# martinambrus/PitchExtractor

Measured on AMD Instinct MI355X. Metric: mel-frames/sec training throughput (JDCNet, 24 kHz, batch=256), higher is better.
Workload: dtype f32

## Files before the change

### include/pitchextractor_hip.h

```cpp
#ifndef PITCHEXTRACTOR_HIP_H
#define PITCHEXTRACTOR_HIP_H

#include <stddef.h>
#include <stdint.h>

#ifdef __cplusplus
extern "C" {
#endif

#define PE_OK 0
#define PE_E_ARG (-1)
#define PE_E_UNSUPPORTED (-2)
#define PE_E_WORKSPACE (-3)

enum pe_products {
  PE_PROD_NATIVE = 0,
  PE_PROD_X3 = 1,
  PE_PROD_H2 = 2,
  PE_PROD_BF16 = 3,
  PE_PROD_F16 = 4
};

int pe_abi_version(void);
int pe_device_count(void);
int pe_stream_create_low_priority(void** stream_out);

typedef struct pe_mel_plan pe_mel_plan;
int pe_mel_plan_create(pe_mel_plan** plan, int sample_rate, int n_fft, int win_length,
                       int hop_length, int n_mels, float f_min, float f_max);
int pe_mel_plan_destroy(pe_mel_plan* plan);
int pe_mel_num_frames(const pe_mel_plan* plan, int n_samples);
int pe_mel_forward(const pe_mel_plan* plan, const float* wave, int batch, int n_samples,
                   long wave_stride, float* out, long out_sb, long out_sm, long out_st,
                   int out_frames, int log_mode, float log_eps, float mean, float std,
                   float pad_value, void* stream);
int pe_mel_forward_ragged(const pe_mel_plan* plan, const float* wave, int batch, int max_samples,
                          long wave_stride, const int* n_samples, const int* frame_start, float* out,
                          long out_sb, long out_sm, long out_st, int out_frames, int log_mode,
                          float log_eps, float mean, float std, float pad_value, void* stream);
int pe_mel_chunk_fields(void);
int pe_mel_forward_chunks(const pe_mel_plan* plan, const float* wave, long wave_elems, const long* chunks,
                          const long* host_chunks, int n_chunks, int chunk_size, float* out, long out_sb,
                          long out_sm, long out_st, int log_mode, float log_eps, float mean, float std,
                          float pad_value, void* stream);
size_t pe_mel_backward_workspace_bytes(const pe_mel_plan* plan, int batch, int max_samples, int out_frames);
int pe_mel_backward(const pe_mel_plan* plan, const float* wave, int batch, int n_samples, long wave_stride,
                    const float* grad_out, long g_sb, long g_sm, long g_st, int out_frames, int log_mode,
                    float log_eps, float mean, float std, float* grad_wave, long grad_wave_stride,
                    void* workspace, size_t workspace_bytes, void* stream);
int pe_mel_backward_ragged(const pe_mel_plan* plan, const float* wave, int batch, int max_samples,
                           long wave_stride, const int* n_samples, const int* frame_start,
                           const float* grad_out, long g_sb, long g_sm, long g_st, int out_frames,
                           int log_mode, float log_eps, float mean, float std, float* grad_wave,
                           long grad_wave_stride, void* workspace, size_t workspace_bytes, void* stream);

int pe_stitch_run_fields(void);
int pe_stitch_chunks(const float* x, long ld_x, const float* det, const long* runs, const long* host_runs,
                     int n_runs, int n_chunks, int chunk_size, int C, float* out, long ld_out, float* det_out,
                     long n_dst, void* stream);


int pe_gemm_nt(int products, int act16, const void* A, long lda, const float* B, long ldb, void* C, long ldc, int M,
               int N, int K, const float* bias0, const float* bias1, int accumulate, const unsigned* amax_a,
               const unsigned* amax_b, void* stream);
int pe_absmax(const float* x, long rows, int cols, long ld, unsigned* out, void* stream);
int pe_absmax_segments(const float* base, const long* seg_off, const long* seg_len, int nseg, unsigned* out,
                       void* stream);
size_t pe_gemm_tn_workspace_bytes(int M, int N, int K);
int pe_gemm_tn(int products, int act16, const void* A, long lda, const void* B, long ldb, float* C, long ldc, int M,
               int N, int K, int accumulate, float* workspace, size_t workspace_bytes, const unsigned* amax_a,
               const unsigned* amax_b, void* stream);
int pe_transpose2d(const float* in, float* out, int rows, int cols, void* stream);

int pe_conv3x3_repack(const float* w_oihw, float* w_fwd, float* w_dgrad, int Cout, int Cin, void* stream);
int pe_conv3x3_fwd(int products, int act16, const void* x, const float* w_packed, void* y, int B, int T, int F, int C,
                   int N, int accumulate, const unsigned* amax_x, const unsigned* amax_w, void* stream);
size_t pe_wfrag_bytes(int products, int N, int K);
int pe_wfrag_pack(int products, const float* w, long ld, int N, int K, const unsigned* amax, void* wfrag, void* stream);
int pe_conv3x3_wf_supported(int F, int C, int N);
int pe_conv3x3_fwd_wf(int products, int act16, const void* x, const void* wfrag, void* y, int B, int T, int F, int C,
                      int N, int accumulate, double* bn_partials, const unsigned* amax_x, const unsigned* amax_w,
                      void* stream);
int pe_conv3x3_wf_stat_parts(int B, int T, int F);
size_t pe_conv3x3_wgrad_workspace_bytes(int B, int T, int F, int Cin, int Cout);
int pe_conv3x3_wgrad(int products, int act16, const void* x, const void* dy, float* dw_oihw, int B, int T, int F,
                     int Cin, int Cout, float* workspace, size_t workspace_bytes, const unsigned* amax_x,
                     const unsigned* amax_dy, void* stream);
int pe_conv3x3_c1_stat_parts(int B, int T, int F);
int pe_conv3x3_c1_fwd(int act16, const float* x, long sb, long st, long sf, const float* w_oihw, void* y, int B, int T,
                      int F, double* bn_partials, void* stream);
int pe_conv3x3_c1_wgrad(int act16, const float* x, long sb, long st, long sf, const void* dy, float* dw_oihw, int B,
                        int T, int F, float* workspace, size_t workspace_bytes, void* stream);
int pe_conv3x3_c1_dgrad(int act16, const void* dy, const float* w_oihw, float* dx, int B, int T, int F, void* stream);

int pe_attn_supported(int T, int dh);
int pe_attn_fwd(int products, const float* qkv, long ld_qkv, float* o, long ld_o, float* lse,
                const unsigned char* mask_in, unsigned char* mask_out, int B, int T, int H, int dh, float scale,
                float p_drop, unsigned long long seed, unsigned long long offset, void* stream);
int pe_attn_bwd(int products, const float* qkv, long ld_qkv, const float* o, const float* d_o, long ld_o,
                const float* lse, const unsigned char* mask, float* dqkv, int B, int T, int H, int dh, float scale,
                float p_drop, void* stream);

size_t pe_bn_workspace_bytes(int C);
int pe_bn_train_stats(int act16, const void* x, long n_pix, int C, const float* gamma, const float* beta, float eps,
                      float momentum, float* running_mean, float* running_var, float* mean, float* invstd,
                      float* scale, float* shift, void* workspace, size_t workspace_bytes, void* stream);
int pe_bn_finalize_stats(const double* partials, int nparts, long n_pix, int C, const float* gamma, const float* beta,
                         float eps, float momentum, float* running_mean, float* running_var, float* mean,
                         float* invstd, float* scale, float* shift, void* workspace, size_t workspace_bytes,
                         void* stream);
int pe_bn_eval_affine(const float* gamma, const float* beta, const float* running_mean,
                      const float* running_var, float eps, int C, float* scale, float* shift, float* mean,
                      float* invstd, void* stream);
int pe_bn_act_pool_fwd(int act16, const void* x, const float* scale, const float* shift, float slope, void* y, long rows,
                       int Fin, int C, int pool, long ldy, int coff, unsigned* amax_out, void* stream);
int pe_bn_act_pool_bwd(int act16, const void* x, const void* dy, const float* scale, const float* shift,
                       const float* mean, const float* invstd, float slope, void* dx, float* dgamma, float* dbeta,
                       long rows, int Fin, int C, int pool, long lddy, int coff, int eval_mode, void* workspace,
                       size_t workspace_bytes, unsigned* amax_out, void* stream);
int pe_maxpool_fwd(int act16, const void* x, void* y, long rows, int Fin, int C, int pool, long ldy, int coff,
                   unsigned char* argmax_out, void* stream);
int pe_maxpool_bwd_add(int act16, const void* x, const unsigned char* argmax, const void* dy, void* dx, long rows,
                       int Fin, int C, int pool, long lddy, int coff, unsigned* amax_out, void* stream);
int pe_bn_act_pool_tap_supported(long rows, int Fin, int C, int pool, int tap_pool, int with_arg);
int pe_bn_act_pool_tap_fwd(int act16, const void* x, const float* scale, const float* shift, float slope, void* y,
                           long rows, int Fin, int C, int pool, long ldy, int coff, unsigned* amax_out, void* tap_y,
                           long tap_ldy, int tap_coff, int tap_pool, unsigned char* tap_arg, void* stream);
int pe_bn_act_pool_tap_bwd(int act16, const void* x, const void* dy, const float* scale, const float* shift,
                           const float* mean, const float* invstd, float slope, void* dx, float* dgamma, float* dbeta,
                           long rows, int Fin, int C, int pool, long lddy, int coff, int eval_mode, void* workspace,
                           size_t workspace_bytes, unsigned* amax_out, const void* tap_dy, long tap_lddy, int tap_coff,
                           int tap_pool, const unsigned char* tap_arg, void* stream);
int pe_dropout_fwd(int act16, const void* x, long ldx, void* y, long ldy, const unsigned char* mask_in,
                   unsigned char* mask_out, long rows, int cols, float p, unsigned long long seed,
                   unsigned long long offset, void* stream);
int pe_nhwc_to_seq(int act16, const void* x, long ldx, int coff, float* seq, long rows, int C, void* stream);
int pe_seq_to_nhwc(int act16, const float* seq, void* x, long ldx, int coff, long rows, int C, int accumulate,
                   void* stream);
int pe_copy2d(int act16, const void* src, long lds, void* dst, long ldd, long rows, int cols, int accumulate,
              void* stream);

int pe_lstm_fwd(int ncells, const float* const* whh, float* const* gates, float* const* y,
                float* const* cbuf, const int* reverse, long ldy, int B, int T, int H, void* stream);
int pe_lstm_bwd(int ncells, const float* const* whh_t, float* const* gates, const float* const* cbuf,
                const float* const* dy, float* const* dcarry, const int* reverse, long lddy, int B, int T,
                int H, void* stream);
size_t pe_lstm_persistent_sync_bytes(int ncells, int B);
int pe_lstm_persistent_supported(int ncells, int B, int H);
int pe_lstm_bwd_persistent_dbias_rows(int ncells, int B, int T, int H, long lddy);
int pe_lstm_fwd_persistent(int products, int ncells, const float* const* whh, float* const* gates, float* const* y,
                           float* const* cbuf, const int* reverse, long ldy, int B, int T, int H, unsigned* sync,
                           void* stream);
int pe_lstm_bwd_persistent(int products, int ncells, const float* const* whh_t, float* const* gates,
                           const float* const* cbuf, const float* const* dy, const int* reverse, long lddy, int B,
                           int T, int H, float* const* dbias_rows, unsigned* const* dgates_amax, unsigned* sync,
                           void* stream);
int pe_lstm_configure_stamps(int enable);
size_t pe_lstm_whh_grad_workspace_bytes(int B, int T, int H);
int pe_lstm_whh_grad(int products, const float* dgates, const float* y, long ldy, float* dwhh, int B, int T, int H,
                     int reverse, float* workspace, size_t workspace_bytes, const unsigned* amax_dgates,
                     const unsigned* amax_y, void* stream);
size_t pe_colsum_workspace_bytes(int cols);
int pe_colsum(const float* x, long rows, int cols, long ld, float* out0, float* out1, void* workspace,
              size_t workspace_bytes, void* stream);

int pe_head_fwd(const float* x, long ldx, const float* w, const float* bias, int n_out, float* y, long R,
                int D, void* stream);
size_t pe_head_bwd_workspace_bytes(int D);
int pe_head_bwd(const float* x, long ldx, const float* w, const float* dy, int n_out, float* dx, long lddx,
                float* dw, float* db, long R, int D, void* workspace, size_t workspace_bytes, void* stream);
int pe_f0_sil_loss(const float* f0_pred, const float* f0, const float* sil_pred, const float* sil,
                   float lambda_f0, long R, float grad_scale, float* out3, float* d_f0_pred,
                   float* d_sil_pred, void* stream);
size_t pe_f0_bins_ce_workspace_bytes(long R);
int pe_f0_bins_ce_loss(const float* logits, long ldl, int C, const float* f0, const float* sil_pred,
                       const float* sil, float lambda_f0, long R, float grad_scale, float* out4,
                       float* d_logits, long ldd, float* d_sil_pred, float* workspace, size_t workspace_bytes,
                       void* stream);
int pe_adamw_step(float* param, const float* grad, float* exp_avg, float* exp_avg_sq, long n, float lr,
                  float beta1, float beta2, float eps, float weight_decay, double bias_correction1,
                  double bias_correction2, float grad_scale, const float* skip_if_nonzero, void* stream);
int pe_nonfinite_flag(const float* x, long n, int* flag, void* stream);


int pe_bgemm(int mode, const float* A, long lda, long a_outer, long a_inner, const float* B, long ldb,
             long b_outer, long b_inner, float* C, long ldc, long c_outer, long c_inner, int inner, int batch,
             int M, int N, int K, float alpha, int accumulate, void* stream);
int pe_softmax_fwd(float* s, long rows, int L, float scale, void* stream);
int pe_softmax_bwd(const float* p, float* dp, long rows, int L, float scale, void* stream);
int pe_layernorm_fwd(const float* a, const float* b, const float* pe, int period, const float* gamma,
                     const float* beta, float eps, float* z_out, float* y, float* mean, float* rstd, long rows,
                     int D, void* stream);
size_t pe_layernorm_bwd_workspace_bytes(int D);
int pe_layernorm_bwd(const float* dy, const float* z, const float* mean, const float* rstd, const float* gamma,
                     float* dz, float* dgamma, float* dbeta, long rows, int D, void* workspace,
                     size_t workspace_bytes, void* stream);
int pe_gelu_fwd(const float* x, float* y, long n, void* stream);
int pe_gelu_bwd(const float* x, const float* dy, float* dx, long n, void* stream);
int pe_layernorm_dropout_fwd(const float* a, const float* b, const float* pe, int period, const float* gamma,
                             const float* beta, float eps, float* z_out, float* y, float* mean, float* rstd,
                             long rows, int D, const unsigned char* mask_in, unsigned char* mask_out, float p,
                             unsigned long long seed, unsigned long long offset, void* stream);
// ... 171 lines not shown
```

### pitchextractor_amd/_lib.py

```python
from __future__ import annotations

import ctypes as C
import os
from pathlib import Path

_PKG = Path(__file__).resolve().parent
LIB_PATH = Path(os.environ.get("PITCHEXTRACTOR_HIP_LIB", _PKG / "libpitchextractor_hip.so"))

_lib = None


class HipLibraryError(RuntimeError):
    pass


_p = C.c_void_p
_i = C.c_int
_l = C.c_long
_f = C.c_float
_d = C.c_double
_z = C.c_size_t
_u64 = C.c_ulonglong
_pp = C.POINTER(C.c_void_p)
_ip = C.POINTER(C.c_int)

PE_PROD_NATIVE, PE_PROD_X3, PE_PROD_H2, PE_PROD_BF16, PE_PROD_F16 = range(5)
PE_F0_ARGMAX, PE_F0_WEIGHTED = range(2)

PROTOTYPES = {
    "pe_abi_version": (_i, []),
    "pe_device_count": (_i, []),
    "pe_stream_create_low_priority": (_i, [C.POINTER(_p)]),
    "pe_mel_plan_create": (_i, [C.POINTER(_p), _i, _i, _i, _i, _i, _f, _f]),
    "pe_mel_plan_destroy": (_i, [_p]),
    "pe_mel_num_frames": (_i, [_p, _i]),
    "pe_mel_forward": (_i, [_p, _p, _i, _i, _l, _p, _l, _l, _l, _i, _i, _f, _f, _f, _f, _p]),
    "pe_mel_forward_ragged": (_i, [_p, _p, _i, _i, _l, _p, _p, _p, _l, _l, _l, _i, _i, _f, _f, _f, _f, _p]),
    "pe_mel_chunk_fields": (_i, []),
    "pe_mel_forward_chunks": (_i, [_p, _p, _l, _p, _p, _i, _i, _p, _l, _l, _l, _i, _f, _f, _f, _f, _p]),
    "pe_mel_backward_workspace_bytes": (_z, [_p, _i, _i, _i]),
    "pe_mel_backward": (_i, [_p, _p, _i, _i, _l, _p, _l, _l, _l, _i, _i, _f, _f, _f, _p, _l, _p, _z, _p]),
    "pe_mel_backward_ragged": (_i, [_p, _p, _i, _i, _l, _p, _p, _p, _l, _l, _l, _i, _i, _f, _f, _f, _p, _l, _p, _z,
                                    _p]),
    "pe_stitch_run_fields": (_i, []),
    "pe_stitch_chunks": (_i, [_p, _l, _p, _p, _p, _i, _i, _i, _i, _p, _l, _p, _l, _p]),
    "pe_gemm_nt": (_i, [_i, _i, _p, _l, _p, _l, _p, _l, _i, _i, _i, _p, _p, _i, _p, _p, _p]),
    "pe_absmax": (_i, [_p, _l, _i, _l, _p, _p]),
    "pe_absmax_segments": (_i, [_p, _p, _p, _i, _p, _p]),
    "pe_gemm_tn_workspace_bytes": (_z, [_i, _i, _i]),
    "pe_gemm_tn": (_i, [_i, _i, _p, _l, _p, _l, _p, _l, _i, _i, _i, _i, _p, _z, _p, _p, _p]),
    "pe_transpose2d": (_i, [_p, _p, _i, _i, _p]),
    "pe_conv3x3_repack": (_i, [_p, _p, _p, _i, _i, _p]),
    "pe_conv3x3_fwd": (_i, [_i, _i, _p, _p, _p, _i, _i, _i, _i, _i, _i, _p, _p, _p]),
    "pe_wfrag_bytes": (_z, [_i, _i, _i]),
    "pe_wfrag_pack": (_i, [_i, _p, _l, _i, _i, _p, _p, _p]),
    "pe_conv3x3_wf_supported": (_i, [_i, _i, _i]),
    "pe_conv3x3_fwd_wf": (_i, [_i, _i, _p, _p, _p, _i, _i, _i, _i, _i, _i, _p, _p, _p, _p]),
    "pe_conv3x3_wgrad_workspace_bytes": (_z, [_i, _i, _i, _i, _i]),
    "pe_conv3x3_wgrad": (_i, [_i, _i, _p, _p, _p, _i, _i, _i, _i, _i, _p, _z, _p, _p, _p]),
    "pe_conv3x3_c1_stat_parts": (_i, [_i, _i, _i]),
    "pe_conv3x3_c1_fwd": (_i, [_i, _p, _l, _l, _l, _p, _p, _i, _i, _i, _p, _p]),
    "pe_conv3x3_c1_wgrad": (_i, [_i, _p, _l, _l, _l, _p, _p, _i, _i, _i, _p, _z, _p]),
    "pe_conv3x3_c1_dgrad": (_i, [_i, _p, _p, _p, _i, _i, _i, _p]),
    "pe_bn_workspace_bytes": (_z, [_i]),
    "pe_bn_train_stats": (_i, [_i, _p, _l, _i, _p, _p, _f, _f, _p, _p, _p, _p, _p, _p, _p, _z, _p]),
    "pe_conv3x3_wf_stat_parts": (_i, [_i, _i, _i]),
    "pe_bn_finalize_stats": (_i, [_p, _i, _l, _i, _p, _p, _f, _f, _p, _p, _p, _p, _p, _p, _p, _z, _p]),
    "pe_bn_eval_affine": (_i, [_p, _p, _p, _p, _f, _i, _p, _p, _p, _p, _p]),
    "pe_bn_act_pool_fwd": (_i, [_i, _p, _p, _p, _f, _p, _l, _i, _i, _i, _l, _i, _p, _p]),
    "pe_bn_act_pool_bwd": (_i, [_i, _p, _p, _p, _p, _p, _p, _f, _p, _p, _p, _l, _i, _i, _i, _l, _i, _i, _p, _z, _p,
                                _p]),
    "pe_maxpool_fwd": (_i, [_i, _p, _p, _l, _i, _i, _i, _l, _i, _p, _p]),
    "pe_maxpool_bwd_add": (_i, [_i, _p, _p, _p, _p, _l, _i, _i, _i, _l, _i, _p, _p]),
    "pe_bn_act_pool_tap_supported": (_i, [_l, _i, _i, _i, _i, _i]),
    "pe_bn_act_pool_tap_fwd": (_i, [_i, _p, _p, _p, _f, _p, _l, _i, _i, _i, _l, _i, _p, _p, _l, _i, _i, _p, _p]),
    "pe_bn_act_pool_tap_bwd": (_i, [_i, _p, _p, _p, _p, _p, _p, _f, _p, _p, _p, _l, _i, _i, _i, _l, _i, _i, _p, _z, _p,
                                    _p, _l, _i, _i, _p, _p]),
    "pe_dropout_fwd": (_i, [_i, _p, _l, _p, _l, _p, _p, _l, _i, _f, _u64, _u64, _p]),
    "pe_nhwc_to_seq": (_i, [_i, _p, _l, _i, _p, _l, _i, _p]),
    "pe_seq_to_nhwc": (_i, [_i, _p, _p, _l, _i, _l, _i, _i, _p]),
    "pe_copy2d": (_i, [_i, _p, _l, _p, _l, _l, _i, _i, _p]),
    "pe_lstm_fwd": (_i, [_i, _pp, _pp, _pp, _pp, _ip, _l, _i, _i, _i, _p]),
    "pe_lstm_bwd": (_i, [_i, _pp, _pp, _pp, _pp, _pp, _ip, _l, _i, _i, _i, _p]),
    "pe_lstm_persistent_sync_bytes": (_z, [_i, _i]),
    "pe_lstm_persistent_supported": (_i, [_i, _i, _i]),
    "pe_lstm_fwd_persistent": (_i, [_i, _i, _pp, _pp, _pp, _pp, _ip, _l, _i, _i, _i, _p, _p]),
    "pe_lstm_bwd_persistent_dbias_rows": (_i, [_i, _i, _i, _i, _l]),
    "pe_lstm_configure_stamps": (_i, [_i]),
    "pe_lstm_bwd_persistent": (_i, [_i, _i, _pp, _pp, _pp, _pp, _ip, _l, _i, _i, _i, _pp, _pp, _p, _p]),
    "pe_lstm_whh_grad_workspace_bytes": (_z, [_i, _i, _i]),
    "pe_lstm_whh_grad": (_i, [_i, _p, _p, _l, _p, _i, _i, _i, _i, _p, _z, _p, _p, _p]),
    "pe_colsum_workspace_bytes": (_z, [_i]),
    "pe_colsum": (_i, [_p, _l, _i, _l, _p, _p, _p, _z, _p]),
    "pe_head_fwd": (_i, [_p, _l, _p, _p, _i, _p, _l, _i, _p]),
    "pe_head_bwd_workspace_bytes": (_z, [_i]),
    "pe_head_bwd": (_i, [_p, _l, _p, _p, _i, _p, _l, _p, _p, _l, _i, _p, _z, _p]),
    "pe_f0_sil_loss": (_i, [_p, _p, _p, _p, _f, _l, _f, _p, _p, _p, _p]),
    "pe_bgemm": (_i, [_i, _p, _l, _l, _l, _p, _l, _l, _l, _p, _l, _l, _l, _i, _i, _i, _i, _i, _f, _i, _p]),
    "pe_attn_supported": (_i, [_i, _i]),
    "pe_attn_fwd": (_i, [_i, _p, _l, _p, _l, _p, _p, _p, _i, _i, _i, _i, _f, _f, _u64, _u64, _p]),
    "pe_attn_bwd": (_i, [_i, _p, _l, _p, _p, _l, _p, _p, _p, _i, _i, _i, _i, _f, _f, _p]),
    "pe_softmax_fwd": (_i, [_p, _l, _i, _f, _p]),
    "pe_softmax_bwd": (_i, [_p, _p, _l, _i, _f, _p]),
    "pe_layernorm_fwd": (_i, [_p, _p, _p, _i, _p, _p, _f, _p, _p, _p, _p, _l, _i, _p]),
    "pe_layernorm_bwd_workspace_bytes": (_z, [_i]),
    "pe_layernorm_bwd": (_i, [_p, _p, _p, _p, _p, _p, _p, _p, _l, _i, _p, _z, _p]),
    "pe_gelu_fwd": (_i, [_p, _p, _l, _p]),
    "pe_gelu_bwd": (_i, [_p, _p, _p, _l, _p]),
    "pe_layernorm_dropout_fwd": (_i, [_p, _p, _p, _i, _p, _p, _f, _p, _p, _p, _p, _l, _i, _p, _p, _f, _u64, _u64, _p]),
    "pe_layernorm_bwd_fused": (_i, [_p, _p, _p, _p, _p, _p, _p, _p, _f, _p, _p, _p, _l, _i, _p, _z, _p]),
    "pe_gelu_dropout_fwd": (_i, [_p, _p, _l, _p, _p, _f, _u64, _u64, _p]),
    "pe_gelu_dropout_bwd": (_i, [_p, _p, _p, _f, _p, _l, _p]),
    "pe_resample_plan_create": (_i, [C.POINTER(_p), _i, _i, _i, _f]),
    "pe_resample_plan_destroy": (_i, [_p]),
    "pe_resample_out_len": (_l, [_p, _l]),
    "pe_resample_forward": (_i, [_p, _p, _i, _i, _l, _p, _l, _i, _p]),
    "pe_resample_ragged_plan_create": (_i, [C.POINTER(_p), _ip, _i, _i, _i, _f]),
    "pe_resample_ragged_plan_destroy": (_i, [_p]),
    "pe_resample_ragged_out_len": (_l, [_p, _i, _l]),
    "pe_resample_ragged_forward": (_i, [_p, _p, _p, _p, _p, _p, _p, _i, _p, _l, _i, _p]),
    "pe_pitch_shift_plan": (_i, [_i, _p, _p, _p, _p, _p, _p, _l, _i, _i, _i, _i, _p, _p, _p]),
    "pe_pitch_shift_plan_fields": (_i, []),
    "pe_pitch_shift_stft": (_i, [_p, _p, _i, _l, _p, _p]),
    "pe_pitch_shift_vocoder": (_i, [_p, _p, _p, _i, _l, _p, _p]),
    "pe_pitch_shift_istft": (_i, [_p, _p, _i, _l, _l, _p, _p, _p]),
    "pe_pitch_shift_resample": (_i, [_p, _p, _p, _p, _i, _p, _p, _i, _l, _p, _p]),
    "pe_world_plan_fields": (_i, []),
    "pe_world_plan": (_i, [_i, _p, _p, _p, _p, _p, _p, _p, _p, _p, _p, _p, _p, _p, _p, _p, _l, _d, _d, _i, _p, _p, _p,
                           _p]),
    "pe_world_responses": (_i, [_p, _p, _p, _p, _p, _p, _p, _i, _l, _i, _p, _p]),
    "pe_world_overlap_add": (_i, [_p, _p, _p, _p, _p, _i, _l, _i, _p, _p]),
    "pe_cheaptrick_plan_fields": (_i, []),
    "pe_cheaptrick_plan": (_i, [_i, _p, _p, _p, _p, _p, _p, _p, _p, _d, _d, _d, _i, _p, _p]),
    "pe_cheaptrick": (_i, [_p, _p, _p, _p, _p, _i, _d, _d, _d, _d, _i, _p, _p]),
    "pe_f0_bins_ce_workspace_bytes": (_z, [_l]),
    "pe_f0_bins_ce_loss": (_i, [_p, _l, _i, _p, _p, _p, _f, _l, _f, _p, _p, _l, _p, _p, _z, _p]),
    "pe_nonfinite_flag": (_i, [_p, _l, _p, _p]),
    "pe_adamw_step": (_i, [_p, _p, _p, _p, _l, _f, _f, _f, _f, _f, _d, _d, _f, _p, _p]),
    "pe_f0_decode_frames": (_i, [_p, _l, _l, _i, _p, _p, _i, _i, _i, _p, _p, _p, _p]),
    "pe_f0_viterbi_workspace_bytes": (_z, [_i, _i, _i]),
    "pe_f0_viterbi": (_i, [_p, _l, _l, _i, _p, _i, _i, _p, _p, _z, _p]),
    "pe_pitch_metrics": (_i, [_p, _p, _l, _d, _p, _p]),
    "pe_f0_track_plan_fields": (_i, []),
    "pe_f0_track_plan": (_i, [_i, _p, _p, _i, _i, _p, _p, _p, _p, _p, _p]),
    "pe_row_stats_workspace_bytes": (_z, [_i]),
# ... 94 lines not shown
```

### pitchextractor_amd/csrc/conv.hip

```cpp
#include <type_traits>
#include "splitk.h"

namespace {
using namespace pe;
typedef unsigned int u32x4_t __attribute__((ext_vector_type(4)));
typedef unsigned int u32x2_t __attribute__((ext_vector_type(2)));

__global__ void repack3x3_kernel(const float* __restrict__ w, float* __restrict__ w_fwd,
                                 float* __restrict__ w_dgrad, int Cout, int Cin) {
  const int idx = blockIdx.x * blockDim.x + threadIdx.x;
  if (idx >= Cout * Cin * 9) return;
  const int tap = idx % 9, ci = (idx / 9) % Cin, co = idx / (9 * Cin);
  const float v = w[idx];
  if (w_fwd) w_fwd[((long)co * 9 + tap) * Cin + ci] = v;
  if (w_dgrad) w_dgrad[((long)ci * 9 + (8 - tap)) * Cout + co] = v;
}

__global__ void transpose2d_kernel(const float* __restrict__ in, float* __restrict__ out, int rows, int cols) {
  __shared__ float tile[32][33];
  const int c0 = blockIdx.x * 32, r0 = blockIdx.y * 32;
  for (int i = threadIdx.y; i < 32; i += 8) {
    const int r = r0 + i, c = c0 + threadIdx.x;
    tile[i][threadIdx.x] = (r < rows && c < cols) ? in[(long)r * cols + c] : 0.f;
  }
  __syncthreads();
  for (int i = threadIdx.y; i < 32; i += 8) {
    const int c = c0 + i, r = r0 + threadIdx.x;
    if (r < rows && c < cols) out[(long)c * rows + r] = tile[threadIdx.x][i];
  }
}

template <class TO>
struct ConvEpiT {
  TO* Y;
  int rows, N, accumulate;
  double* stats;
  int buffer;
  __device__ __forceinline__ void operator()(int row, int col, float v) const {
    if (row < rows && col < N) {
      TO* d = Y + (long)row * N + col;
      if (accumulate) v += ld1(d);
      st1(d, v);
    }
  }
};
typedef ConvEpiT<float> ConvEpi;

template <class TO> __device__ __forceinline__ float stored_value(float v) {
  if constexpr (std::is_same<TO, float>::value) return v;
  else return __uint_as_float(pack_bf16_rne(v, 0.f) << 16);
}

template <class TL, int MODE, class TA = float, class TH = __bf16>
__global__ __launch_bounds__(256) void conv3x3_kernel(ConvLoader<TL::A_LOADS, TA> al, RowLoader bl, ConvEpiT<TA> ep,
                                                      int K, int tiles_m, int tiles_n, const unsigned* amax_x,
                                                      const unsigned* amax_w) {
  __shared__ __attribute__((aligned(16))) float As[TL::BM * nt_row_floats<MODE>()];
  __shared__ __attribute__((aligned(16))) float Bs[TL::BN * nt_row_floats<MODE>()];
  const int tile = xcd_remap(blockIdx.x, tiles_m * tiles_n);
  const int m0 = (tile / tiles_n) * TL::BM, n0 = (tile % tiles_n) * TL::BN;
  al.init(m0);
  bl.init(n0);
  f32x16 acc[TL::TM][TL::TN];
  zero_acc<TL>(acc);
  H2Scales hs{1.f, 1.f, 1.f};
  if constexpr (MODE == kSplit2) hs.load(amax_x, amax_w);
  nt_mainloop_mode<TL, MODE, false, 1, TH>(al, bl, K, As, Bs, acc, hs.sa, hs.sb);
  for_each_acc<TL>(acc, [&](int r, int c, float v) { ep(m0 + r, n0 + c, MODE == kSplit2 ? hs.unscale(v) : v); });
}

template <class TL, class FM, class TA = typename FM::TA>
int launch_conv(const TA* x, const float* wp, TA* y, int B, int T, int F, int C, int N, int accumulate,
                hipStream_t st, const unsigned* amax_x, const unsigned* amax_w) {
  const int rows = B * T * F, K = 9 * C;
  ConvLoader<TL::A_LOADS, TA> al;
  al.p = x; al.T = T; al.F = F; al.C = C; al.rows = rows;
  RowLoader bl{wp, (long)K, N, K, 0};
  ConvEpiT<TA> ep{y, rows, N, accumulate, nullptr};
  const int tm = pe_cdiv(rows, TL::BM), tn = pe_cdiv(N, TL::BN);
  hipLaunchKernelGGL((conv3x3_kernel<TL, FM::MODE, TA, typename FM::TH>), dim3(tm * tn), dim3(256), 0, st, al, bl, ep, K,
                     tm, tn, amax_x, amax_w);
  PE_LAUNCH_CHECK();
  return PE_OK;
}


template <int NT, class TH = __bf16>
__global__ void wfrag_pack_kernel(const float* __restrict__ w, long ld, int N, int K, uint4* __restrict__ out,
                                  const unsigned* __restrict__ amax = nullptr) {
  const long idx = (long)blockIdx.x * blockDim.x + threadIdx.x;
  const int NB32 = (N + 31) >> 5, KB = K >> 4;
  const int lane = (int)(idx & 63);
  const long blk = idx >> 6;
  if (blk >= (long)NB32 * KB) return;
  const int nb = (int)(blk % NB32), kb = (int)(blk / NB32);
  const int n = nb * 32 + (lane & 31), k = kb * 16 + (lane >> 5) * 8;
  float4 v0 = make_float4(0.f, 0.f, 0.f, 0.f), v1 = v0;
  if (n < N) {
    v0 = *reinterpret_cast<const float4*>(w + (long)n * ld + k);
    v1 = *reinterpret_cast<const float4*>(w + (long)n * ld + k + 4);
  }
  uint4* dst = out + ((long)(kb * NB32 + nb) * NT) * 64 + lane;
  if constexpr (NT == 3) {
    const Split3 a = split3(v0), b = split3(v1);
    dst[0] = make_uint4(a.hi.x, a.hi.y, b.hi.x, b.hi.y);
    dst[64] = make_uint4(a.mid.x, a.mid.y, b.mid.x, b.mid.y);
    dst[128] = make_uint4(a.lo.x, a.lo.y, b.lo.x, b.lo.y);
  } else if constexpr (NT == 2) {
    const float sc = h2_scale(*amax);
    const Split2 a = split2(v0, sc), b = split2(v1, sc);
    dst[0] = make_uint4(a.hi.x, a.hi.y, b.hi.x, b.hi.y);
    dst[64] = make_uint4(a.lo.x, a.lo.y, b.lo.x, b.lo.y);
  } else {
    const half4<TH> a = to_half4<TH>(v0), b = to_half4<TH>(v1);
    const uint2 ua = __builtin_bit_cast(uint2, a), ub = __builtin_bit_cast(uint2, b);
    dst[0] = make_uint4(ua.x, ua.y, ub.x, ub.y);
  }
}

template <int BN, int MODE, int PASSES, int D, bool FA2, class TA = float, class TH = __bf16>
__global__ __launch_bounds__(256, 2) void conv3x3_halo_wf_kernel(const TA* __restrict__ x,
                                                                 const uint4* __restrict__ wf, ConvEpiT<TA> ep, int T,
                                                                 int F, int C, int N, int P, int tiles_m,
                                                                 int tiles_n, const unsigned* amax_x,
                                                                 const unsigned* amax_w) {
  constexpr int NT = mode_terms<MODE>();
  using H = term_t<NT, TH>;
  H2Scales hs{1.f, 1.f, 1.f};
  if constexpr (MODE == kSplit2) hs.load(amax_x, amax_w);
  constexpr int TM = 2, TN = BN / 64, WN = BN / 2;
  constexpr int ZR = PASSES * 32;
  constexpr int AIMG = (ZR + 4) * 32;
  constexpr int S = 18 * TN;
  static_assert(S % D == 0 && D >= 2, "the fragment ring wraps at chunk boundaries");
// ... 469 lines not shown
    }
#pragma unroll
    for (int kk = 0; kk < kBK / 16; ++kk) {
      half8<H> fa[NT];
#pragma unroll
      for (int c = 0; c < NT; ++c) fa[c] = tr_fragment(a_rd + c * YIMG + kk * 16 * ST, ST);
#pragma unroll
      for (int w = 0; w < 3; ++w)
#pragma unroll
        for (int d = 0; d < 3; ++d) {
          const H* rd[2];
#pragma unroll
          for (int e = 0; e < 2; ++e) {
            const int j = 2 * kk + e;
            const bool ok = (w == 1 || tv[j][w >> 1]) && (d == 1 || fv[j][d >> 1]);
            rd[e] = ok ? b_rd + (w * WS + kk * 16 + 4 * e + d) * ST : z_rd;
          }
          half8<H> fb[NT];
#pragma unroll
          for (int c = 0; c < NT; ++c) {
            const s16x4 lo = lds_read_tr(rd[0] + c * XIMG), hi = lds_read_tr(rd[1] + c * XIMG);
            typedef short s16x8 __attribute__((ext_vector_type(8)));
            const s16x8 v = {lo[0], lo[1], lo[2], lo[3], hi[0], hi[1], hi[2], hi[3]};
            fb[c] = __builtin_bit_cast(half8<H>, v);
          }
          acc[w * 3 + d] = mfma_terms<NT>(fa, fb, acc[w * 3 + d]);
        }
    }
#pragma unroll
    for (int j = 0; j < 4; ++j) {
      fj[j] += f_step;
      tj[j] += t_step;
      if (fj[j] >= F) { fj[j] -= F; ++tj[j]; }
      if (tj[j] >= T) tj[j] -= T;
    }
  }
#pragma unroll
  for (int tp = 0; tp < 9; ++tp) {
    float* dst = ws + ((long)split_id * 9 + tp) * Cout * Cin;
#pragma unroll
    for (int q = 0; q < 16; ++q) {
      const int co = m0 + wm * 32 + (q & 3) + 8 * (q >> 2) + 4 * h;
      const int ci = n0 + wn * 32 + r;
      dst[(long)co * Cin + ci] = NT == 2 ? hs.unscale(acc[tp][q]) : acc[tp][q];
    }
  }
}

static inline bool wgrad9_halo(int F) { return 2 * F + 34 <= 80; }

struct OihwDst {
  float* dw;
  int Cout, Cin;
  __host__ __device__ long elems() const { return 9L * Cout * Cin; }
  __device__ __forceinline__ void operator()(long i4, const float4& s) const {
    const int idx = (int)i4 * 4;
    const int ci = idx % Cin, co = (idx / Cin) % Cout, tap = idx / (Cin * Cout);
    float* d = dw + ((long)co * Cin + ci) * 9 + tap;
    d[0] = s.x; d[9] = s.y; d[18] = s.z; d[27] = s.w;
  }
};

bool wgrad9_ok(int Cout, int Cin) { return (Cout % 64) == 0 && (Cin % 64) == 0; }

struct WgradPlan { int bm, bn; SplitK k; };

WgradPlan wgrad_plan(int P, int Cout, int Cin) {
  const bool nine = wgrad9_ok(Cout, Cin);
  const int bm = (nine || Cout <= 64) ? 64 : 128, bn = (nine || Cin <= 64) ? 64 : 128;
  const int tiles = pe_cdiv(Cout, bm) * pe_cdiv(Cin, bn) * (nine ? 1 : 9);
  return {bm, bn, splitk_plan(tiles, P, 1024, resident_wgs(nine ? 2 : 3))};
}

template <int BM, int BN>
void launch_wgrad(const float* x, const float* dy, float* ws, int T, int F, int Cin, int Cout, int P, SplitK k,
                 hipStream_t st) {
  const int tm = pe_cdiv(Cout, BM), tn = pe_cdiv(Cin, BN);
  const int n_tiles = tm * tn, n_chunks = n_tiles * k.splits;
  const int grid = 8 * 9 * pe_cdiv(n_chunks, 8);
  hipLaunchKernelGGL((conv3x3_wgrad_kernel<BM, BN>), dim3(grid), dim3(256), 0, st, dy, x, ws, T, F, Cin, Cout, P, k.kps,
                     tn, n_tiles, n_chunks);
}

template <bool STATS, class TA = float>
__global__ __launch_bounds__(256) void conv3x3_c1_fwd_kernel(const float* __restrict__ x, long sb, long st_, long sf,
                                                             const float* __restrict__ w, TA* __restrict__ y,
                                                             double* __restrict__ bn_partials, int B, int T, int F) {
  __shared__ double sred[STATS ? 2 * 16 * 64 : 1];
  double s1[4] = {0.0, 0.0, 0.0, 0.0}, s2[4] = {0.0, 0.0, 0.0, 0.0};
  const int q = threadIdx.x & 15;
  float wr[4][9];
#pragma unroll
  for (int c = 0; c < 4; ++c)
#pragma unroll
    for (int k = 0; k < 9; ++k) wr[c][k] = w[(q * 4 + c) * 9 + k];
  const int F4 = F >> 2, R = B * T * F4;
  for (int run = blockIdx.x * 16 + (threadIdx.x >> 4); run < R; run += gridDim.x * 16) {
    const int bt = run / F4, f0 = (run - bt * F4) * 4;
    const long b = bt / T;
    const int t = bt - (int)b * T;
    float in[3][6];
#pragma unroll
    for (int dt = 0; dt < 3; ++dt)
#pragma unroll
      for (int df = 0; df < 6; ++df) {
        const int tt = t + dt - 1, ff = f0 + df - 1;
        in[dt][df] = (tt >= 0 && tt < T && ff >= 0 && ff < F) ? x[b * sb + tt * st_ + ff * sf] : 0.f;
      }
#pragma unroll
    for (int px = 0; px < 4; ++px) {
      float4 o;
      float* op = reinterpret_cast<float*>(&o);
#pragma unroll
      for (int c = 0; c < 4; ++c) {
        float s = 0.f;
#pragma unroll
        for (int k = 0; k < 9; ++k) s = fmaf(in[k / 3][px + k % 3], wr[c][k], s);
        op[c] = s;
        if constexpr (STATS) {
          const double dv = (double)stored_value<TA>(s);
          s1[c] += dv;
          s2[c] += dv * dv;
        }
      }
      st4(y + ((long)bt * F + f0 + px) * 64 + q * 4, o);
    }
  }
  if constexpr (STATS) {
    const int grp = threadIdx.x >> 4;
#pragma unroll
    for (int c = 0; c < 4; ++c) {
      sred[grp * 64 + q * 4 + c] = s1[c];
      sred[16 * 64 + grp * 64 + q * 4 + c] = s2[c];
    }
    __syncthreads();
    if (threadIdx.x < 128) {
      const int which = threadIdx.x >> 6, ch = threadIdx.x & 63;
      double t = 0.0;
#pragma unroll
      for (int g = 0; g < 16; ++g) t += sred[which * 16 * 64 + g * 64 + ch];
      bn_partials[((long)blockIdx.x * 2 + which) * 64 + ch] = t;
    }
  }
}

template <class TA = float>
__global__ __launch_bounds__(256) void conv3x3_c1_wgrad_kernel(const float* __restrict__ x, long sb, long st_,
                                                               long sf, const TA* __restrict__ dy,
                                                               float* __restrict__ partial, int B, int T, int F) {
  __shared__ float red[16][64][9];
  const int q = threadIdx.x & 15, grp = threadIdx.x >> 4;
  float acc[4][9];
#pragma unroll
  for (int c = 0; c < 4; ++c)
#pragma unroll
    for (int k = 0; k < 9; ++k) acc[c][k] = 0.f;
  const int F4 = F >> 2, R = B * T * F4;
  for (int run = blockIdx.x * 16 + grp; run < R; run += gridDim.x * 16) {
    const int bt = run / F4, f0 = (run - bt * F4) * 4, b = bt / T, t = bt - b * T;
    const float* xb = x + b * sb;
    float in[3][6];
#pragma unroll
    for (int dt = 0; dt < 3; ++dt)
#pragma unroll
      for (int df = 0; df < 6; ++df) {
        const int tt = t + dt - 1, ff = f0 + df - 1;
        in[dt][df] = (tt >= 0 && tt < T && ff >= 0 && ff < F) ? xb[tt * st_ + ff * sf] : 0.f;
      }
#pragma unroll
    for (int px = 0; px < 4; ++px) {
      const float4 g = ld4(dy + ((long)bt * F + f0 + px) * 64 + q * 4);
#pragma unroll
      for (int k = 0; k < 9; ++k) {
        const float xv = in[k / 3][px + k % 3];
        acc[0][k] = fmaf(g.x, xv, acc[0][k]);
        acc[1][k] = fmaf(g.y, xv, acc[1][k]);
        acc[2][k] = fmaf(g.z, xv, acc[2][k]);
        acc[3][k] = fmaf(g.w, xv, acc[3][k]);
      }
    }
  }
#pragma unroll
  for (int c = 0; c < 4; ++c)
#pragma unroll
    for (int k = 0; k < 9; ++k) red[grp][q * 4 + c][k] = acc[c][k];
  __syncthreads();
  for (int i = threadIdx.x; i < 64 * 9; i += 256) {
    const int c = i / 9, k = i % 9;
    float s = 0.f;
#pragma unroll
    for (int gq = 0; gq < 16; ++gq) s += red[gq][c][k];
    partial[(long)blockIdx.x * 576 + i] = s;
  }
}

__global__ void c1_wgrad_reduce_kernel(const float* __restrict__ partial, float* __restrict__ dw, int nblocks) {
  const int i = blockIdx.x * 4 + (threadIdx.x >> 6);
  if (i >= 576) return;
  const int lane = threadIdx.x & 63;
  double s = 0.0;
  for (int z = lane; z < nblocks; z += 64) s += (double)partial[(long)z * 576 + i];
#pragma unroll
  for (int off = 32; off > 0; off >>= 1) s += __shfl_down(s, off, 64);
  if (lane == 0) dw[i] = (float)s;
}

template <int CTRL>
__device__ __forceinline__ float dpp_move(float v) {
  return __int_as_float(__builtin_amdgcn_update_dpp(0, __float_as_int(v), CTRL, 0xf, 0xf, true));
}
constexpr int kDppSwap1 = 0xB1, kDppSwap2 = 0x4E;
constexpr int kDppRor8 = 0x128, kDppRor4 = 0x124;

constexpr int kDgTT = 30, kDgTF = 16, kDgHF = kDgTF + 2, kDgHalo = (kDgTT + 2) * kDgHF;
static_assert(kDgHalo % 64 == 0, "whole passes of 16 groups x 4 pixels");

template <class TA>
__global__ __launch_bounds__(256) void conv3x3_c1_dgrad_kernel(const TA* __restrict__ dy, const float* __restrict__ w,
                                                               float* __restrict__ dx, int T, int F, int tiles_t,
                                                               int tiles_f) {
  __shared__ float part[kDgHalo * 9];
  const int lane = threadIdx.x & 15, grp = threadIdx.x >> 4;
  float wr[4][9];
#pragma unroll
  for (int c = 0; c < 4; ++c)
#pragma unroll
    for (int k = 0; k < 9; ++k) wr[c][k] = w[(lane * 4 + c) * 9 + k];
  const int tf = blockIdx.x % tiles_f, tt = (blockIdx.x / tiles_f) % tiles_t, b = blockIdx.x / (tiles_f * tiles_t);
  const int t0 = tt * kDgTT, f0 = tf * kDgTF;
  const TA* dyb = dy + (long)b * T * F * 64 + lane * 4;
  const bool odd1 = lane & 1, odd2 = lane & 2;
  for (int q = grp; q < kDgHalo / 4; q += 16) {
    float4 g[4];
#pragma unroll
    for (int u = 0; u < 4; ++u) {
      const int h = q * 4 + u, hr = h / kDgHF, t = t0 - 1 + hr, f = f0 - 1 + (h - hr * kDgHF);
      g[u] = (t >= 0 && t < T && f >= 0 && f < F) ? ld4(dyb + ((long)t * F + f) * 64) : make_float4(0.f, 0.f, 0.f, 0.f);
    }
    float s[9];
#pragma unroll
    for (int k = 0; k < 9; ++k) {
      float a[4];
#pragma unroll
      for (int u = 0; u < 4; ++u)
        a[u] = fmaf(g[u].w, wr[3][k], fmaf(g[u].z, wr[2][k], fmaf(g[u].y, wr[1][k], g[u].x * wr[0][k])));
      const float p0 = (odd1 ? a[2] : a[0]) + dpp_move<kDppSwap1>(odd1 ? a[0] : a[2]);
      const float p1 = (odd1 ? a[3] : a[1]) + dpp_move<kDppSwap1>(odd1 ? a[1] : a[3]);
      float v = (odd2 ? p1 : p0) + dpp_move<kDppSwap2>(odd2 ? p0 : p1);
      v += dpp_move<kDppRor8>(v);
      s[k] = v + dpp_move<kDppRor4>(v);
    }
    if (lane < 4) {
      float* pp = part + (q * 4 + 2 * (lane & 1) + (lane >> 1)) * 9;
#pragma unroll
// ... 96 lines not shown
                               const unsigned* amax_w) {
  constexpr int MODE = FM::MODE;
  if (!x || !wfrag || !y || B <= 0 || T <= 0 || F <= 0 || C <= 0 || N <= 0) return PE_E_ARG;
  if ((C % 32) != 0 || (long)B * T * F * (C > N ? C : N) >= (1L << 31)) return PE_E_UNSUPPORTED;
  if ((long)B * T * F * C * (long)sizeof(TA) >= (1L << 31) || (long)pe_wfrag_bytes_host(N, 9 * C, mode_terms<MODE>()) >= (1L << 31))
    return PE_E_UNSUPPORTED;
  if (MODE == kSplit2 && (!amax_x || !amax_w)) return PE_E_ARG;
  hipStream_t st = pe_stream(stream);
  const int passes = conv_halo_passes(F, N);
  if (passes == 10)
    return launch_conv_halo_wf<64, FM, 10, 6, true>(x, wfrag, y, B, T, F, C, N, accumulate, stats, st, amax_x, amax_w);
  if (passes == 7) {
    if (N % 192 == 0 && N % 128 != 0)
      return launch_conv_halo_wf<192, FM, 7, 3, false>(x, wfrag, y, B, T, F, C, N, accumulate, stats, st, amax_x,
                                                       amax_w);
    return launch_conv_halo_wf<128, FM, 7, 3, true>(x, wfrag, y, B, T, F, C, N, accumulate, stats, st, amax_x, amax_w);
  }
  return PE_E_UNSUPPORTED;
}

extern "C" int pe_conv3x3_fwd_wf(int products, int act16, const void* x, const void* wfrag, void* y, int B, int T, int F,
                                 int C, int N, int accumulate, double* bn_partials, const unsigned* amax_x,
                                 const unsigned* amax_w, void* stream) {
  return with_form<kTermForms, true>(products, act16, [&](auto f) {
    using TA = typename decltype(f)::TA;
    return conv3x3_fwd_wf_impl<decltype(f)>(static_cast<const TA*>(x), wfrag, static_cast<TA*>(y), B, T, F, C, N,
                                            accumulate, bn_partials, stream, amax_x, amax_w);
  });
}

extern "C" size_t pe_conv3x3_wgrad_workspace_bytes(int B, int T, int F, int Cin, int Cout) {
  if (Cin == 1) return (size_t)kC1WgradBlocks * 576 * sizeof(float);
  return (size_t)wgrad_plan(B * T * F, Cout, Cin).k.splits * 9 * Cout * Cin * sizeof(float);
}

template <class FM, class TA = typename FM::TA>
static int conv3x3_wgrad_impl(const TA* x, const TA* dy, float* dw_oihw, int B, int T, int F, int Cin,
                              int Cout, float* workspace, size_t workspace_bytes, void* stream,
                              const unsigned* amax_x, const unsigned* amax_dy) {
  constexpr int MODE = FM::MODE;
  using TH = typename FM::TH;
  if (!x || !dy || !dw_oihw || B <= 0 || T <= 0 || F <= 0 || Cin <= 0 || Cout <= 0) return PE_E_ARG;
  if (MODE == kSplit2 && (!amax_x || !amax_dy)) return PE_E_ARG;
  if ((Cin & 3) || (Cout & 3)) return PE_E_UNSUPPORTED;
  if (!workspace || workspace_bytes < pe_conv3x3_wgrad_workspace_bytes(B, T, F, Cin, Cout)) return PE_E_WORKSPACE;
  const int P = B * T * F;
  const WgradPlan pl = wgrad_plan(P, Cout, Cin);
  const SplitK k = pl.k;
  hipStream_t st = pe_stream(stream);
  if (wgrad9_ok(Cout, Cin)) {
    const int tn = Cin / 64;
    const dim3 grid((Cout / 64) * tn * k.splits);
    if constexpr (MODE != kNative) {
      constexpr int NT = mode_terms<MODE>();
      hipLaunchKernelGGL((wgrad9_halo(F) ? conv3x3_wgrad9_x3_kernel<NT, true, TA, TH>
                                         : conv3x3_wgrad9_x3_kernel<NT, false, TA, TH>),
                         grid, dim3(256), 0, st, dy, x, workspace, T, F, Cin, Cout, P, k.kps, tn, amax_dy, amax_x);
    } else {
      hipLaunchKernelGGL(conv3x3_wgrad9_kernel<0>, grid, dim3(256), 0, st, dy, x, workspace, T, F, Cin, Cout, P, k.kps,
                         tn);
    }
  } else if constexpr (std::is_same<TA, float>::value) {
    if (pl.bm == 64 && pl.bn == 64) launch_wgrad<64, 64>(x, dy, workspace, T, F, Cin, Cout, P, k, st);
    else if (pl.bm == 64) launch_wgrad<64, 128>(x, dy, workspace, T, F, Cin, Cout, P, k, st);
    else if (pl.bn == 64) launch_wgrad<128, 64>(x, dy, workspace, T, F, Cin, Cout, P, k, st);
    else launch_wgrad<128, 128>(x, dy, workspace, T, F, Cin, Cout, P, k, st);
  } else {
    return PE_E_UNSUPPORTED;
  }
  PE_LAUNCH_CHECK();
  return launch_splitk_reduce(workspace, k.splits, OihwDst{dw_oihw, Cout, Cin}, st);
}

extern "C" int pe_conv3x3_wgrad(int products, int act16, const void* x, const void* dy, float* dw_oihw, int B, int T, int F,
                                int Cin, int Cout, float* workspace, size_t workspace_bytes, const unsigned* amax_x,
                                const unsigned* amax_dy, void* stream) {
  return with_form<kAllForms, true>(products, act16, [&](auto f) {
    using TA = typename decltype(f)::TA;
    return conv3x3_wgrad_impl<decltype(f)>(static_cast<const TA*>(x), static_cast<const TA*>(dy), dw_oihw, B, T, F, Cin,
                                           Cout, workspace, workspace_bytes, stream, amax_x, amax_dy);
  });
}

static int c1_grid(int B, int T, int F) {
  const long R = (long)B * T * (F / 4);
  return (int)((R + 15) / 16 < 8192 ? (R + 15) / 16 : 8192);
}

extern "C" int pe_conv3x3_c1_stat_parts(int B, int T, int F) { return (B > 0 && T > 0 && F > 0) ? c1_grid(B, T, F) : 0; }

template <class TA>
static int conv3x3_c1_fwd_impl(const float* x, long sb, long st, long sf, const float* w_oihw, TA* y, int B, int T,
                               int F, double* bn_partials, void* stream) {
  if (!x || !w_oihw || !y || B <= 0 || T <= 0 || F <= 0) return PE_E_ARG;
  if ((F & 3) || (long)B * T * F >= (1L << 31) - 64L * 8192) return PE_E_UNSUPPORTED;
  const int grid = c1_grid(B, T, F);
  if (bn_partials)
    hipLaunchKernelGGL((conv3x3_c1_fwd_kernel<true, TA>), dim3(grid), dim3(256), 0, pe_stream(stream), x, sb, st, sf,
                       w_oihw, y, bn_partials, B, T, F);
  else
    hipLaunchKernelGGL((conv3x3_c1_fwd_kernel<false, TA>), dim3(grid), dim3(256), 0, pe_stream(stream), x, sb, st, sf,
                       w_oihw, y, nullptr, B, T, F);
  PE_LAUNCH_CHECK();
  return PE_OK;
}

extern "C" int pe_conv3x3_c1_fwd(int act16, const float* x, long sb, long st, long sf, const float* w_oihw, void* y, int B,
                                 int T, int F, double* bn_partials, void* stream) {
  return with_act(act16, [&](auto a) {
    using TA = typename decltype(a)::TA;
    return conv3x3_c1_fwd_impl(x, sb, st, sf, w_oihw, static_cast<TA*>(y), B, T, F, bn_partials, stream);
  });
}

template <class TA>
static int conv3x3_c1_wgrad_impl(const float* x, long sb, long st, long sf, const TA* dy, float* dw_oihw, int B, int T,
                                 int F, float* workspace, size_t workspace_bytes, void* stream) {
  if (!x || !dy || !dw_oihw || B <= 0 || T <= 0 || F <= 0) return PE_E_ARG;
  if ((F & 3) || (long)B * T * F >= (1L << 31) - 65536) return PE_E_UNSUPPORTED;
  if (!workspace || workspace_bytes < (size_t)kC1WgradBlocks * 576 * sizeof(float)) return PE_E_WORKSPACE;
  hipLaunchKernelGGL(conv3x3_c1_wgrad_kernel<TA>, dim3(kC1WgradBlocks), dim3(256), 0, pe_stream(stream), x, sb, st, sf,
                     dy, workspace, B, T, F);
  PE_LAUNCH_CHECK();
  hipLaunchKernelGGL(c1_wgrad_reduce_kernel, dim3(144), dim3(256), 0, pe_stream(stream), workspace, dw_oihw,
                     kC1WgradBlocks);
  PE_LAUNCH_CHECK();
  return PE_OK;
}

extern "C" int pe_conv3x3_c1_wgrad(int act16, const float* x, long sb, long st, long sf, const void* dy, float* dw_oihw,
                                   int B, int T, int F, float* workspace, size_t workspace_bytes, void* stream) {
  return with_act(act16, [&](auto a) {
    using TA = typename decltype(a)::TA;
    return conv3x3_c1_wgrad_impl(x, sb, st, sf, static_cast<const TA*>(dy), dw_oihw, B, T, F, workspace, workspace_bytes,
                                 stream);
  });
}

template <class TA>
static int conv3x3_c1_dgrad_impl(const TA* dy, const float* w_oihw, float* dx, int B, int T, int F, void* stream) {
  if (!dy || !w_oihw || !dx || B <= 0 || T <= 0 || F <= 0) return PE_E_ARG;
  if ((F & 3) || (long)B * T * F >= (1L << 31) - 65536) return PE_E_UNSUPPORTED;
  const int tiles_t = (T + kDgTT - 1) / kDgTT, tiles_f = (F + kDgTF - 1) / kDgTF;
  hipLaunchKernelGGL(conv3x3_c1_dgrad_kernel<TA>, dim3(B * tiles_t * tiles_f), dim3(256), 0, pe_stream(stream), dy,
                     w_oihw, dx, T, F, tiles_t, tiles_f);
  PE_LAUNCH_CHECK();
  return PE_OK;
}

extern "C" int pe_conv3x3_c1_dgrad(int act16, const void* dy, const float* w_oihw, float* dx, int B, int T, int F,
                                   void* stream) {
  if (act16 == 2) return conv3x3_c1_dgrad_impl(static_cast<const _Float16*>(dy), w_oihw, dx, B, T, F, stream);
  return with_act(act16, [&](auto a) {
    using TA = typename decltype(a)::TA;
    return conv3x3_c1_dgrad_impl(static_cast<const TA*>(dy), w_oihw, dx, B, T, F, stream);
  });
}
```

### pitchextractor_amd/csrc/elementwise.hip

```cpp
#include <type_traits>
#include "forms.h"

namespace {
using namespace pe;

constexpr int kMaxPartials = 4096;

template <class F>
__device__ __forceinline__ void column_reduce2(F&& f, long n_pix, int C, double* partial ) {
  extern __shared__ __attribute__((aligned(16))) char smem_raw[];
  double* red = reinterpret_cast<double*>(smem_raw);
  const int quads = C >> 2;
  const int G = 256 / quads;
  const int q = threadIdx.x % quads, g = threadIdx.x / quads;
  double s1[4] = {0, 0, 0, 0}, s2[4] = {0, 0, 0, 0};
  if (g < G) {
    for (long p = (long)blockIdx.x * G + g; p < n_pix; p += (long)gridDim.x * G) {
      float4 a, b;
      f(p, q * 4, a, b);
      s1[0] += a.x; s1[1] += a.y; s1[2] += a.z; s1[3] += a.w;
      s2[0] += b.x; s2[1] += b.y; s2[2] += b.z; s2[3] += b.w;
    }
#pragma unroll
    for (int i = 0; i < 4; ++i) {
      red[(g * 2 + 0) * C + q * 4 + i] = s1[i];
      red[(g * 2 + 1) * C + q * 4 + i] = s2[i];
    }
  }
  __syncthreads();
  for (int i = threadIdx.x; i < 2 * C; i += 256) {
    double s = 0;
    for (int gg = 0; gg < G; ++gg) s += red[gg * 2 * C + i];
    partial[(long)blockIdx.x * 2 * C + i] = s;
  }
}

__device__ __forceinline__ float lrelu(float v, float slope) { return v > 0.f ? v : v * slope; }

__device__ __forceinline__ float4 bn_lrelu4(const float4& v, const float4& sc, const float4& sh, float slope) {
  return make_float4(lrelu(fmaf(v.x, sc.x, sh.x), slope), lrelu(fmaf(v.y, sc.y, sh.y), slope),
                     lrelu(fmaf(v.z, sc.z, sh.z), slope), lrelu(fmaf(v.w, sc.w, sh.w), slope));
}

__device__ __forceinline__ float4 fmax4(const float4& a, const float4& b) {
  return make_float4(fmaxf(a.x, b.x), fmaxf(a.y, b.y), fmaxf(a.z, b.z), fmaxf(a.w, b.w));
}

__device__ __forceinline__ float4 bn_dx4(const float4& dz, const float4& v, const float4& mu, const float4& is,
                                         const float4& sc, const float4& k1, const float4& k2) {
  return make_float4(sc.x * (dz.x - k1.x - (v.x - mu.x) * is.x * k2.x), sc.y * (dz.y - k1.y - (v.y - mu.y) * is.y * k2.y),
                     sc.z * (dz.z - k1.z - (v.z - mu.z) * is.z * k2.z), sc.w * (dz.w - k1.w - (v.w - mu.w) * is.w * k2.w));
}

__device__ __forceinline__ void first_max(float& m, int& at, float x, int pos, bool force = false) {
  if (force || x > m) { m = x; at = pos; }
}

struct FirstMax4 {
  float4 v;
  int p0, p1, p2, p3;

  __device__ __forceinline__ static FirstMax4 at(const float4& x, int pos) { return FirstMax4{x, pos, pos, pos, pos}; }

  __device__ __forceinline__ void take(const float4& x, int pos, bool force = false) {
    first_max(v.x, p0, x.x, pos, force);
    first_max(v.y, p1, x.y, pos, force);
    first_max(v.z, p2, x.z, pos, force);
    first_max(v.w, p3, x.w, pos, force);
  }

  template <class TA>
  __device__ __forceinline__ static FirstMax4 scan(const TA* xp, long stride, int n) {
    FirstMax4 m = at(ld4(xp), 0);
    int j = 1;
    for (; j + 4 <= n; j += 4) {
      float4 x[4];
#pragma unroll
      for (int u = 0; u < 4; ++u) x[u] = ld4(xp + (long)(j + u) * stride);
#pragma unroll
      for (int u = 0; u < 4; ++u) m.take(x[u], j + u);
    }
    for (; j < n; ++j) m.take(ld4(xp + (long)j * stride), j);
    return m;
  }

  __device__ __forceinline__ uchar4 bytes() const {
    return make_uchar4((unsigned char)p0, (unsigned char)p1, (unsigned char)p2, (unsigned char)p3);
  }
};

template <class TA>
__global__ __launch_bounds__(256) void bn_stats_partial_kernel(const TA* __restrict__ x, long n_pix, int C,
                                                               double* __restrict__ partial) {
  column_reduce2(
      [&](long p, int c, float4& a, float4& b) {
        a = ld4(x + p * C + c);
        b = make_float4(a.x * a.x, a.y * a.y, a.z * a.z, a.w * a.w);
      },
      n_pix, C, partial);
}

__global__ __launch_bounds__(256) void bn_partials_fold_kernel(const double* __restrict__ partial, int nparts, int C2,
                                                               double* __restrict__ out) {
  for (int col = threadIdx.x; col < C2; col += 256) {
    double s = 0.0;
    for (int p = blockIdx.x; p < nparts; p += gridDim.x) s += partial[(long)p * C2 + col];
    out[(long)blockIdx.x * C2 + col] = s;
  }
}

__global__ void bn_stats_finalize_kernel(const double* __restrict__ partial, int nparts, long n_pix, int C,
                                         const float* __restrict__ gamma, const float* __restrict__ beta, float eps,
                                         float momentum, float* __restrict__ running_mean,
                                         float* __restrict__ running_var, float* __restrict__ mean_out,
                                         float* __restrict__ invstd_out, float* __restrict__ scale,
                                         float* __restrict__ shift) {
  const int c = blockIdx.x * 4 + (threadIdx.x >> 6);
  if (c >= C) return;
  const double s1 = pe_wave_strided_sum(partial + c, 2L * C, nparts);
  const double s2 = pe_wave_strided_sum(partial + C + c, 2L * C, nparts);
  if ((threadIdx.x & 63) != 0) return;
  const double n = (double)n_pix;
  const double mean = s1 / n;
  double var = s2 / n - mean * mean;
  if (var < 0) var = 0;
  const float invstd = (float)(1.0 / sqrt(var + (double)eps));
  mean_out[c] = (float)mean;
  invstd_out[c] = invstd;
  const float sc = gamma[c] * invstd;
  scale[c] = sc;
  shift[c] = beta[c] - (float)mean * sc;
  if (running_mean) {
    const double unbiased = n > 1 ? var * n / (n - 1.0) : var;
    running_mean[c] = (1.f - momentum) * running_mean[c] + momentum * (float)mean;
    running_var[c] = (1.f - momentum) * running_var[c] + momentum * (float)unbiased;
  }
}

__global__ void bn_eval_affine_kernel(const float* __restrict__ gamma, const float* __restrict__ beta,
                                      const float* __restrict__ rm, const float* __restrict__ rv, float eps, int C,
                                      float* __restrict__ scale, float* __restrict__ shift,
                                      float* __restrict__ mean, float* __restrict__ invstd_out) {
  const int c = blockIdx.x * blockDim.x + threadIdx.x;
  if (c >= C) return;
  const float invstd = 1.0f / sqrtf(rv[c] + eps);
  const float sc = gamma[c] * invstd;
  scale[c] = sc;
  shift[c] = beta[c] - rm[c] * sc;
  mean[c] = rm[c];
  invstd_out[c] = invstd;
}

__device__ __forceinline__ float amax4(float m, const float4& v) {
  return fmaxf(m, fmaxf(fmaxf(fabsf(v.x), fabsf(v.y)), fmaxf(fabsf(v.z), fabsf(v.w))));
}

__device__ __forceinline__ void amax_commit(float m, unsigned* __restrict__ amax) {
  if (amax == nullptr) return;
#pragma unroll
  for (int off = 32; off > 0; off >>= 1) m = fmaxf(m, __shfl_xor(m, off, 64));
  __shared__ float amax_red[4];
  if ((threadIdx.x & 63) == 0) amax_red[threadIdx.x >> 6] = m;
  __syncthreads();
  if (threadIdx.x == 0) {
    const float w = fmaxf(fmaxf(amax_red[0], amax_red[1]), fmaxf(amax_red[2], amax_red[3]));
    atomicMax(amax, __float_as_uint(w));
  }
}

template <class TA>
__global__ __launch_bounds__(256) void bn_act_pool_fwd_kernel(const TA* __restrict__ x,
                                                              const float* __restrict__ scale,
                                                              const float* __restrict__ shift, float slope,
                                                              TA* __restrict__ y, long n_out_pix, int Fin, int C,
                                                              int pool, long ldy, int coff,
                                                              unsigned* __restrict__ amax) {
  const int quads = C >> 2;
  const int Fout = Fin / pool;
  float am = 0.f;
  const int G = 256 / quads, q = threadIdx.x % quads, g = threadIdx.x / quads;
  const float4 sc = *reinterpret_cast<const float4*>(scale + q * 4), sh = *reinterpret_cast<const float4*>(shift + q * 4);
  for (long op = (long)blockIdx.x * G + g; g < G && op < n_out_pix; op += (long)gridDim.x * G) {
    const long row = op / Fout;
    const int fo = (int)(op % Fout);
    const TA* xp = x + ((row * Fin + (long)fo * pool) * C + q * 4);
    float4 m;
    for (int j = 0; j < pool; ++j) {
      const float4 a = bn_lrelu4(ld4(xp + (long)j * C), sc, sh, slope);
      m = j == 0 ? a : fmax4(m, a);
    }
    st4(y + op * ldy + coff + q * 4, m);
    am = amax4(am, m);
  }
  amax_commit(am, amax);
}

template <int POOL, class TA>
__global__ __launch_bounds__(256) void bn_act_pool_tap_fwd_kernel(const TA* __restrict__ x,
                                                                  const float* __restrict__ scale,
                                                                  const float* __restrict__ shift, float slope,
                                                                  TA* __restrict__ y, long n_tap, int C, int nbw, int S,
                                                                  long ldy, int coff, unsigned* __restrict__ amax,
                                                                  TA* __restrict__ tap_y, long tap_ldy, int tap_coff,
                                                                  unsigned char* __restrict__ tap_arg) {
  __shared__ float4 tap_val[2][256];
  __shared__ uchar4 tap_pos[2][256];
  const int quads = C >> 2;
  const int G = 256 / quads, q = threadIdx.x % quads, g = threadIdx.x / quads;
  const int TW = G / S, segw = nbw / S;
  const int wl = g / S, seg = g - wl * S;
  const bool lane_on = g < TW * S;
  const float4 sc = *reinterpret_cast<const float4*>(scale + q * 4), sh = *reinterpret_cast<const float4*>(shift + q * 4);
  const long n_trips = (n_tap + TW - 1) / TW;
  float am = 0.f;
  int buf = 0;
  for (long trip = blockIdx.x; trip < n_trips; trip += gridDim.x, buf ^= 1) {
    const long tw = trip * TW + wl;
    const bool on = lane_on && tw < n_tap;
    const float ninf = -__builtin_inff();
    FirstMax4 tm = FirstMax4::at(make_float4(ninf, ninf, ninf, ninf), seg * segw * POOL);
    if (on) {
      const long op0 = tw * nbw + (long)seg * segw;
      const TA* xp = x + (op0 * POOL * C + q * 4);
      TA* yp = y + (op0 * ldy + coff + q * 4);
      int pos = seg * segw * POOL;
      bool first = seg == 0;
      for (int i = 0; i < segw; ++i, xp += (long)POOL * C, yp += ldy) {
        float4 v[POOL];
#pragma unroll
        for (int j = 0; j < POOL; ++j) v[j] = ld4(xp + (long)j * C);
        float4 m;
#pragma unroll
        for (int j = 0; j < POOL; ++j, ++pos) {
          const float4 a = bn_lrelu4(v[j], sc, sh, slope);
          m = j == 0 ? a : fmax4(m, a);
          tm.take(v[j], pos, first);
          first = false;
        }
        st4(yp, m);
        am = amax4(am, m);
      }
      if (S > 1) {
        tap_val[buf][threadIdx.x] = tm.v;
        tap_pos[buf][threadIdx.x] = tm.bytes();
      }
    }
    if (S > 1) __syncthreads();
    if (on && seg == 0) {
      for (int k = 1; k < S; ++k) {
        const float4 o = tap_val[buf][threadIdx.x + k * quads];
        const uchar4 p = tap_pos[buf][threadIdx.x + k * quads];
        if (o.x > tm.v.x) { tm.v.x = o.x; tm.p0 = p.x; }
        if (o.y > tm.v.y) { tm.v.y = o.y; tm.p1 = p.y; }
        if (o.z > tm.v.z) { tm.v.z = o.z; tm.p2 = p.z; }
        if (o.w > tm.v.w) { tm.v.w = o.w; tm.p3 = p.w; }
      }
      st4(tap_y + tw * tap_ldy + tap_coff + q * 4, tm.v);
      if (tap_arg != nullptr) *reinterpret_cast<uchar4*>(tap_arg + tw * C + q * 4) = tm.bytes();
    }
  }
  amax_commit(am, amax);
}

template <class TA>
struct BnBwdArgsT {
  const TA* x;
  const TA* dy;
  const float* scale;
  const float* shift;
  const float* mean;
  const float* invstd;
  float slope;
  long n_in_pix;
  int Fin, C;
  long lddy;
// ... 1 lines not shown
};

__global__ void bn_bwd_finalize_kernel(const double* __restrict__ partial, int nparts, long n_pix, int C,
                                       float* __restrict__ dgamma, float* __restrict__ dbeta,
                                       float* __restrict__ c1, float* __restrict__ c2) {
  const int c = blockIdx.x * 4 + (threadIdx.x >> 6);
  if (c >= C) return;
  const double s1 = pe_wave_strided_sum(partial + c, 2L * C, nparts);
  const double s2 = pe_wave_strided_sum(partial + C + c, 2L * C, nparts);
  if ((threadIdx.x & 63) != 0) return;
  dbeta[c] = (float)s1;
  dgamma[c] = (float)s2;
  if (c1 == nullptr) return;
  c1[c] = (float)(s1 / (double)n_pix);
  c2[c] = (float)(s2 / (double)n_pix);
}

__device__ __forceinline__ float4 bn_term(const float* __restrict__ k, int c) {
  return k != nullptr ? *reinterpret_cast<const float4*>(k + c) : make_float4(0.f, 0.f, 0.f, 0.f);
}

template <int POOL>
struct BnWindow {
  float4 v[POOL], dz[POOL];
  long p0;
  int n;
};

template <int POOL, class TA>
__device__ __forceinline__ void bn_window(const BnBwdArgsT<TA>& a, long item, int nwin, int c, BnWindow<POOL>& w,
                                          const float4& sc, const float4& sh) {
  const int Fout = a.Fin / POOL;
  const long row = item / nwin;
  const int wi = (int)(item - row * nwin);
  const bool real = wi < Fout;
  w.n = real ? POOL : a.Fin - Fout * POOL;
  w.p0 = row * a.Fin + (long)wi * POOL;
  const TA* xp = a.x + w.p0 * a.C + c;
#pragma unroll
  for (int j = 0; j < POOL; ++j) {
    w.v[j] = j < w.n ? ld4(xp + (long)j * a.C) : make_float4(0.f, 0.f, 0.f, 0.f);
    w.dz[j] = make_float4(0.f, 0.f, 0.f, 0.f);
  }
  if (!real) return;
  const float4 dyv = ld4(a.dy + (row * Fout + wi) * a.lddy + a.coff + c);
  const float scv[4] = {sc.x, sc.y, sc.z, sc.w}, shv[4] = {sh.x, sh.y, sh.z, sh.w};
  const float dys[4] = {dyv.x, dyv.y, dyv.z, dyv.w};
#pragma unroll
  for (int ch = 0; ch < 4; ++ch) {
    float best = lrelu(fmaf(reinterpret_cast<const float*>(&w.v[0])[ch], scv[ch], shv[ch]), a.slope);
    int arg = 0;
#pragma unroll
    for (int j = 1; j < POOL; ++j)
      first_max(best, arg, lrelu(fmaf(reinterpret_cast<const float*>(&w.v[j])[ch], scv[ch], shv[ch]), a.slope), j);
    const float g = best > 0.f ? dys[ch] : dys[ch] * a.slope;
#pragma unroll
    for (int j = 0; j < POOL; ++j) reinterpret_cast<float*>(&w.dz[j])[ch] = j == arg ? g : 0.f;
  }
}

template <int POOL, class TA>
__global__ __launch_bounds__(256) void bn_bwd_partial_win_kernel(const BnBwdArgsT<TA> a, long n_items, int nwin,
                                                                 double* __restrict__ partial) {
  const int c0 = (threadIdx.x % (a.C >> 2)) * 4;
  const float4 mu = *reinterpret_cast<const float4*>(a.mean + c0), is = *reinterpret_cast<const float4*>(a.invstd + c0);
  const float4 sc = *reinterpret_cast<const float4*>(a.scale + c0), sh = *reinterpret_cast<const float4*>(a.shift + c0);
  column_reduce2(
      [&](long item, int c, float4& s, float4& t) {
        BnWindow<POOL> w;
        bn_window<POOL, TA>(a, item, nwin, c, w, sc, sh);
        s = make_float4(0.f, 0.f, 0.f, 0.f);
        t = make_float4(0.f, 0.f, 0.f, 0.f);
#pragma unroll
        for (int j = 0; j < POOL; ++j) {
          s.x += w.dz[j].x; s.y += w.dz[j].y; s.z += w.dz[j].z; s.w += w.dz[j].w;
          t.x += w.dz[j].x * ((w.v[j].x - mu.x) * is.x); t.y += w.dz[j].y * ((w.v[j].y - mu.y) * is.y);
          t.z += w.dz[j].z * ((w.v[j].z - mu.z) * is.z); t.w += w.dz[j].w * ((w.v[j].w - mu.w) * is.w);
        }
      },
      n_items, a.C, partial);
}

template <class TA>
struct BnTapGrad {
  const TA* dy;
  const unsigned char* arg;
  long lddy;
  int coff;
  unsigned nbw;
};

__device__ __forceinline__ float round_act(const float*, float v) { return v; }
__device__ __forceinline__ float round_act(const act16_t*, float v) {
  return __uint_as_float(pack_bf16_rne(v, 0.f) << 16);
}
__device__ __forceinline__ float add_unfused(float a, float b) {
#pragma clang fp contract(off)
  return a + b;
}

struct NoTap {};

template <int POOL, class TA, class Tap>
__device__ __forceinline__ void bn_bwd_apply_win(const BnBwdArgsT<TA>& a, long n_items, int nwin,
                                                 const float* __restrict__ c1, const float* __restrict__ c2,
                                                 TA* __restrict__ dx, unsigned* __restrict__ amax, const Tap& t) {
  constexpr bool TAP = !std::is_same<Tap, NoTap>::value;
  const int quads = a.C >> 2;
  float am = 0.f;
  const int G = 256 / quads, c = (threadIdx.x % quads) * 4, g = threadIdx.x / quads;
  const float4 mu = *reinterpret_cast<const float4*>(a.mean + c), is = *reinterpret_cast<const float4*>(a.invstd + c);
  const float4 sc = *reinterpret_cast<const float4*>(a.scale + c), sh = *reinterpret_cast<const float4*>(a.shift + c);
  const float4 k1 = bn_term(c1, c), k2 = bn_term(c2, c);
  for (long item = (long)blockIdx.x * G + g; g < G && item < n_items; item += (long)gridDim.x * G) {
    BnWindow<POOL> w;
    bn_window<POOL, TA>(a, item, nwin, c, w, sc, sh);
    [[maybe_unused]] int pos0 = 0;
    [[maybe_unused]] uchar4 ar;
    [[maybe_unused]] float4 tg;
    if constexpr (TAP) {
      const unsigned tw = (unsigned)item / t.nbw;
      pos0 = (int)((unsigned)item - tw * t.nbw) * POOL;
      ar = *reinterpret_cast<const uchar4*>(t.arg + (long)tw * a.C + c);
      tg = ld4(t.dy + (long)tw * t.lddy + t.coff + c);
    }
#pragma unroll
    for (int j = 0; j < POOL; ++j) {
      if (j >= w.n) break;
      float4 o = bn_dx4(w.dz[j], w.v[j], mu, is, sc, k1, k2);
      am = amax4(am, o);
      if constexpr (TAP) {
        const int pj = pos0 + j;
        if (ar.x == pj) { o.x = add_unfused(round_act(dx, o.x), tg.x); am = fmaxf(am, fabsf(o.x)); }
        if (ar.y == pj) { o.y = add_unfused(round_act(dx, o.y), tg.y); am = fmaxf(am, fabsf(o.y)); }
        if (ar.z == pj) { o.z = add_unfused(round_act(dx, o.z), tg.z); am = fmaxf(am, fabsf(o.z)); }
        if (ar.w == pj) { o.w = add_unfused(round_act(dx, o.w), tg.w); am = fmaxf(am, fabsf(o.w)); }
      }
      st4(dx + (w.p0 + j) * a.C + c, o);
    }
  }
  amax_commit(am, amax);
}

template <int POOL, class TA>
__global__ __launch_bounds__(256) void bn_bwd_apply_win_kernel(const BnBwdArgsT<TA> a, long n_items, int nwin,
                                                               const float* __restrict__ c1,
                                                               const float* __restrict__ c2, TA* __restrict__ dx,
                                                               unsigned* __restrict__ amax) {
  bn_bwd_apply_win<POOL, TA>(a, n_items, nwin, c1, c2, dx, amax, NoTap{});
}

template <int POOL, class TA>
__global__ __launch_bounds__(256) void bn_bwd_apply_win_tap_kernel(const BnBwdArgsT<TA> a, long n_items, int nwin,
                                                                   const float* __restrict__ c1,
                                                                   const float* __restrict__ c2, TA* __restrict__ dx,
                                                                   unsigned* __restrict__ amax, const BnTapGrad<TA> t) {
  bn_bwd_apply_win<POOL, TA>(a, n_items, nwin, c1, c2, dx, amax, t);
}

template <class TA>
__global__ __launch_bounds__(256) void maxpool_fwd_kernel(const TA* __restrict__ x, TA* __restrict__ y,
                                                          long n_out_pix, int Fin, int C, int pool, long ldy,
                                                          int coff, unsigned char* __restrict__ arg) {
  const int quads = C >> 2, Fout = Fin / pool;
  const long total = n_out_pix * quads;
  for (long i = (long)blockIdx.x * 256 + threadIdx.x; i < total; i += (long)gridDim.x * 256) {
    const int q = (int)(i % quads);
    const long op = i / quads, row = op / Fout;
    const int fo = (int)(op % Fout);
    const TA* xp = x + ((row * Fin + (long)fo * pool) * C + q * 4);
    float4 m = ld4(xp);
    int a0 = 0, a1 = 0, a2 = 0, a3 = 0;
    const auto take = [&](const float4& v, int pos) {
      first_max(m.x, a0, v.x, pos);
      first_max(m.y, a1, v.y, pos);
      first_max(m.z, a2, v.z, pos);
      first_max(m.w, a3, v.w, pos);
    };
// ... 256 lines not shown
  hipLaunchKernelGGL(bn_eval_affine_kernel, dim3(pe_cdiv(C, 64)), dim3(64), 0, pe_stream(stream), gamma, beta,
                     running_mean, running_var, eps, C, scale, shift, mean, invstd);
  PE_LAUNCH_CHECK();
  return PE_OK;
}

template <class TA>
static int bn_act_pool_fwd_impl(const TA* x, const float* scale, const float* shift, float slope, TA* y, long rows,
                                int Fin, int C, int pool, long ldy, int coff, unsigned* amax_out, void* stream) {
  if (!x || !scale || !shift || !y || rows <= 0 || Fin <= 0 || pool <= 0) return PE_E_ARG;
  if (!bn_channels_ok(C) || (ldy & 3) || (coff & 3)) return PE_E_UNSUPPORTED;
  const long n_out = rows * (Fin / pool);
  hipLaunchKernelGGL(bn_act_pool_fwd_kernel<TA>, dim3(ew_grid(pe_cdiv(n_out, 256 / (C / 4)) * 256L)), dim3(256), 0, pe_stream(stream), x,
                     scale, shift, slope, y, n_out, Fin, C, pool, ldy, coff, amax_out);
  PE_LAUNCH_CHECK();
  return PE_OK;
}

extern "C" int pe_bn_act_pool_fwd(int act16, const void* x, const float* scale, const float* shift, float slope, void* y,
                                  long rows, int Fin, int C, int pool, long ldy, int coff, unsigned* amax_out,
                                  void* stream) {
  return with_act(act16, [&](auto a) {
    using TA = typename decltype(a)::TA;
    return bn_act_pool_fwd_impl(static_cast<const TA*>(x), scale, shift, slope, static_cast<TA*>(y), rows, Fin, C, pool,
                                ldy, coff, amax_out, stream);
  });
}

template <class TA>
static int bn_act_pool_bwd_impl(const TA* x, const TA* dy, const float* scale, const float* shift, const float* mean,
                                const float* invstd, float slope, TA* dx, float* dgamma, float* dbeta, long rows,
                                int Fin, int C, int pool, long lddy, int coff, int eval_mode, void* workspace,
                                size_t workspace_bytes, unsigned* amax_out, void* stream,
                                const BnTapGrad<TA>* tap = nullptr) {
  const bool sums = !(eval_mode && !dgamma && !dbeta);
  if (!x || !dy || !scale || !shift || !mean || !invstd || !dx || rows <= 0) return PE_E_ARG;
  if (sums && (!dgamma || !dbeta)) return PE_E_ARG;
  if (!bn_channels_ok(C) || (lddy & 3) || (coff & 3)) return PE_E_UNSUPPORTED;
  const size_t need = pe_bn_workspace_bytes(C) + 2 * (size_t)C * sizeof(float);
  if (sums && (!workspace || workspace_bytes < need)) return PE_E_WORKSPACE;
  hipStream_t st = pe_stream(stream);
  const BnBwdArgsT<TA> a{x, dy, scale, shift, mean, invstd, slope, rows * Fin, Fin, C, lddy, coff};
  double* partial = reinterpret_cast<double*>(workspace);
  float* c1 = eval_mode ? nullptr
                        : reinterpret_cast<float*>(reinterpret_cast<char*>(workspace) + pe_bn_workspace_bytes(C));
  float* c2 = eval_mode ? nullptr : c1 + C;
  return with_pool(pool, [&](auto p) {
    constexpr int POOL = decltype(p)::value;
    const int nwin = Fin / POOL + (Fin % POOL ? 1 : 0);
    const long n_items = rows * nwin;
    if (sums) {
      const int grid = reduce_grid(n_items, C, (!std::is_same<TA, float>::value && POOL == 1) ? kMaxPartials : 1024);
      hipLaunchKernelGGL((bn_bwd_partial_win_kernel<POOL, TA>), dim3(grid), dim3(256), reduce_lds(C), st, a, n_items,
                         nwin, partial);
      PE_LAUNCH_CHECK();
      hipLaunchKernelGGL(bn_bwd_finalize_kernel, dim3(pe_cdiv(C, 4)), dim3(256), 0, st, partial, grid, a.n_in_pix, C,
                         dgamma, dbeta, c1, c2);
      PE_LAUNCH_CHECK();
    }
    const dim3 agrid(ew_grid(pe_cdiv(n_items, 256 / (C / 4)) * 256L));
    if (tap != nullptr)
      hipLaunchKernelGGL((bn_bwd_apply_win_tap_kernel<POOL, TA>), agrid, dim3(256), 0, st, a, n_items, nwin, c1, c2, dx,
                         amax_out, *tap);
    else
      hipLaunchKernelGGL((bn_bwd_apply_win_kernel<POOL, TA>), agrid, dim3(256), 0, st, a, n_items, nwin, c1, c2, dx,
                         amax_out);
    PE_LAUNCH_CHECK();
    return (int)PE_OK;
  });
}

extern "C" int pe_bn_act_pool_bwd(int act16, const void* x, const void* dy, const float* scale, const float* shift,
                                  const float* mean, const float* invstd, float slope, void* dx, float* dgamma,
                                  float* dbeta, long rows, int Fin, int C, int pool, long lddy, int coff, int eval_mode,
                                  void* workspace, size_t workspace_bytes, unsigned* amax_out, void* stream) {
  return with_act(act16, [&](auto a) {
    using TA = typename decltype(a)::TA;
    return bn_act_pool_bwd_impl(static_cast<const TA*>(x), static_cast<const TA*>(dy), scale, shift, mean, invstd, slope,
                                static_cast<TA*>(dx), dgamma, dbeta, rows, Fin, C, pool, lddy, coff, eval_mode,
                                workspace, workspace_bytes, amax_out, stream);
  });
}

static bool tap_geometry_ok(long rows, int Fin, int C, int pool, int tap_pool, bool with_arg) {
  if (!bn_channels_ok(C) || rows <= 0 || Fin <= 0) return false;
  if (pool != 1 && pool != 2 && pool != 4) return false;
  if (tap_pool <= 0 || tap_pool % pool != 0 || Fin % tap_pool != 0) return false;
  if (with_arg && tap_pool > 255) return false;
  return rows * (long)Fin < (1L << 31);
}

extern "C" int pe_bn_act_pool_tap_supported(long rows, int Fin, int C, int pool, int tap_pool, int with_arg) {
  return tap_geometry_ok(rows, Fin, C, pool, tap_pool, with_arg != 0) ? 1 : 0;
}

template <class TA>
static int bn_act_pool_tap_fwd_impl(const TA* x, const float* scale, const float* shift, float slope, TA* y, long rows,
                                    int Fin, int C, int pool, long ldy, int coff, unsigned* amax_out, TA* tap_y,
                                    long tap_ldy, int tap_coff, int tap_pool, unsigned char* tap_arg, void* stream) {
  if (!x || !scale || !shift || !y || !tap_y || rows <= 0 || Fin <= 0 || pool <= 0) return PE_E_ARG;
  if ((ldy & 3) || (coff & 3) || (tap_ldy & 3) || (tap_coff & 3) ||
      !tap_geometry_ok(rows, Fin, C, pool, tap_pool, tap_arg != nullptr))
    return PE_E_UNSUPPORTED;
  const int G = 256 / (C / 4), nbw = tap_pool / pool;
  int S = 1, used = 0;
  for (int s = 1; s <= G && s <= nbw; ++s) {
    if (nbw % s) continue;
    const int u = (G / s) * s;
    if (u >= used) { used = u; S = s; }
  }
  const long n_tap = rows * (Fin / tap_pool), n_trips = pe_cdiv(n_tap, (long)(G / S));
  const dim3 grid(ew_grid(n_trips * 256L));
  hipStream_t st = pe_stream(stream);
  return with_pool(pool, [&](auto p) {
    hipLaunchKernelGGL((bn_act_pool_tap_fwd_kernel<decltype(p)::value, TA>), grid, dim3(256), 0, st, x, scale, shift,
                       slope, y, n_tap, C, nbw, S, ldy, coff, amax_out, tap_y, tap_ldy, tap_coff, tap_arg);
    PE_LAUNCH_CHECK();
    return (int)PE_OK;
  });
}

extern "C" int pe_bn_act_pool_tap_fwd(int act16, const void* x, const float* scale, const float* shift, float slope,
                                      void* y, long rows, int Fin, int C, int pool, long ldy, int coff,
                                      unsigned* amax_out, void* tap_y, long tap_ldy, int tap_coff, int tap_pool,
                                      unsigned char* tap_arg, void* stream) {
  return with_act(act16, [&](auto a) {
    using TA = typename decltype(a)::TA;
    return bn_act_pool_tap_fwd_impl(static_cast<const TA*>(x), scale, shift, slope, static_cast<TA*>(y), rows, Fin, C,
                                    pool, ldy, coff, amax_out, static_cast<TA*>(tap_y), tap_ldy, tap_coff, tap_pool,
                                    tap_arg, stream);
  });
}

extern "C" int pe_bn_act_pool_tap_bwd(int act16, const void* x, const void* dy, const float* scale, const float* shift,
                                      const float* mean, const float* invstd, float slope, void* dx, float* dgamma,
                                      float* dbeta, long rows, int Fin, int C, int pool, long lddy, int coff,
                                      int eval_mode, void* workspace, size_t workspace_bytes, unsigned* amax_out,
                                      const void* tap_dy,
                                      long tap_lddy, int tap_coff, int tap_pool, const unsigned char* tap_arg,
                                      void* stream) {
  return with_act(act16, [&](auto a) {
    using TA = typename decltype(a)::TA;
    if (!tap_dy || !tap_arg) return (int)PE_E_ARG;
    if ((tap_lddy & 3) || (tap_coff & 3) || !tap_geometry_ok(rows, Fin, C, pool, tap_pool, true))
      return (int)PE_E_UNSUPPORTED;
    const BnTapGrad<TA> tap{static_cast<const TA*>(tap_dy), tap_arg, tap_lddy, tap_coff, (unsigned)(tap_pool / pool)};
    return bn_act_pool_bwd_impl(static_cast<const TA*>(x), static_cast<const TA*>(dy), scale, shift, mean, invstd, slope,
                                static_cast<TA*>(dx), dgamma, dbeta, rows, Fin, C, pool, lddy, coff, eval_mode,
                                workspace, workspace_bytes, amax_out, stream, &tap);
  });
}

template <class TA>
static int maxpool_fwd_impl(const TA* x, TA* y, long rows, int Fin, int C, int pool, long ldy, int coff,
                            unsigned char* argmax_out, void* stream) {
  if (!x || !y || rows <= 0 || Fin <= 0 || pool <= 0) return PE_E_ARG;
  if ((C & 3) || (ldy & 3) || (coff & 3) || (argmax_out && pool > 255)) return PE_E_UNSUPPORTED;
  const long n_out = rows * (Fin / pool);
  hipLaunchKernelGGL(maxpool_fwd_kernel<TA>, dim3(ew_grid(n_out * (C / 4))), dim3(256), 0, pe_stream(stream), x, y,
                     n_out, Fin, C, pool, ldy, coff, argmax_out);
  PE_LAUNCH_CHECK();
  return PE_OK;
}

extern "C" int pe_maxpool_fwd(int act16, const void* x, void* y, long rows, int Fin, int C, int pool, long ldy, int coff,
                              unsigned char* argmax_out, void* stream) {
// ... 125 lines not shown
```

### pitchextractor_amd/csrc/lib.hip

```cpp
#include "common.h"

extern "C" int pe_abi_version(void) { return 7; }

extern "C" int pe_device_count(void) {
  int n = 0;
  hipError_t e = hipGetDeviceCount(&n);
  if (e != hipSuccess) return -(int)e;
  return n;
}

extern "C" int pe_stream_create_low_priority(void** stream_out) {
  if (!stream_out) return PE_E_ARG;
  int least = 0, greatest = 0;
  PE_CHECK_HIP(hipDeviceGetStreamPriorityRange(&least, &greatest));
  hipStream_t st = nullptr;
  PE_CHECK_HIP(hipStreamCreateWithPriority(&st, hipStreamNonBlocking, least));
  *stream_out = reinterpret_cast<void*>(st);
  return PE_OK;
}
```

### pitchextractor_amd/model.py

```python
from __future__ import annotations

import math
import os

import torch
from torch import nn
from torch.autograd.function import once_differentiable

from . import ops

_ALIGN = 4


class _Conv(nn.Module):

    def __init__(self, cin, cout, k):
        super().__init__()
        self.weight = nn.Parameter(torch.empty(cout, cin, k, k))


class _BatchNorm(nn.Module):
    def __init__(self, c, eps=1e-5, momentum=0.1):
        super().__init__()
        self.eps, self.momentum = eps, momentum
# ... 53 lines not shown
        pe = torch.zeros(max_len, d_model)
        position = torch.arange(0, max_len, dtype=torch.float).unsqueeze(1)
        div_term = torch.exp(torch.arange(0, d_model, 2).float() * (-math.log(10000.0) / d_model))
        pe[:, 0::2] = torch.sin(position * div_term)
        pe[:, 1::2] = torch.cos(position * div_term)
        self.register_buffer("pe", pe.unsqueeze(0))


class _LayerNorm(nn.Module):
    def __init__(self, d, eps=1e-5):
        super().__init__()
        self.eps = eps
        self.weight = nn.Parameter(torch.ones(d))
        self.bias = nn.Parameter(torch.zeros(d))


class _SelfAttention(nn.Module):
    def __init__(self, d, nhead):
        super().__init__()
        self.embed_dim, self.num_heads = d, nhead
        self.in_proj_weight = nn.Parameter(torch.empty(3 * d, d))
        self.in_proj_bias = nn.Parameter(torch.zeros(3 * d))
        self.out_proj = _Linear(d, d)


class _EncoderLayer(nn.Module):

    def __init__(self, d, nhead, ff, dropout):
        super().__init__()
        self.p = dropout
        self.self_attn = _SelfAttention(d, nhead)
        self.linear1 = _Linear(d, ff)
        self.linear2 = _Linear(ff, d)
        self.norm1 = _LayerNorm(d)
        self.norm2 = _LayerNorm(d)


class _Encoder(nn.Module):
    def __init__(self, d, nhead, ff, dropout, num_layers):
        super().__init__()
        self.layers = nn.ModuleList([_EncoderLayer(d, nhead, ff, dropout) for _ in range(num_layers)])


class SequenceModel(nn.Module):

    def __init__(self, input_size, model_type="bilstm", hidden_size=384, num_layers=2, dropout=0.3,
                 bidirectional=True, nhead=8, dim_feedforward=1024, max_len=2000):
        super().__init__()
        self.model_type = model_type.lower()
        self.input_size, self.hidden_size = input_size, hidden_size
        self.bidirectional, self.num_layers = bidirectional, num_layers
        if self.model_type == "bilstm":
            self.dropout = dropout if num_layers > 1 else 0.0
            self.model = _LSTMWeights(input_size, hidden_size, num_layers, bidirectional)
            self._output_dim = hidden_size * (2 if bidirectional else 1)
        elif self.model_type == "transformer":
            if input_size not in (256, 512, 768, 1024) or input_size % nhead or (input_size // nhead) % 4:
                raise NotImplementedError("transformer head: d_model must be 256/512/768/1024 and divide by nhead")
            self.dropout = dropout
            self.nhead, self.dim_feedforward = nhead, dim_feedforward
            self.pos_encoding = SinusoidalPositionalEncoding(input_size, max_len=max_len)
            self.model = _Encoder(input_size, nhead, dim_feedforward, dropout, num_layers)
            self.layer_norm = _LayerNorm(input_size)
            self._output_dim = input_size
        else:
            raise ValueError(f"Unsupported sequence model type: {model_type}")

    @property
    def output_dim(self):
        return self._output_dim


class _Linear(nn.Module):
    def __init__(self, d_in, d_out):
        super().__init__()
        self.weight = nn.Parameter(torch.empty(d_out, d_in))
        self.bias = nn.Parameter(torch.zeros(d_out))


class _Ctx:
    """Tensors one forward pass leaves behind for its backward."""


def _bn(mod: _BatchNorm, x, train: bool, partials=None):
    if train:
        st = ops.bn_train_stats(x, mod.weight, mod.bias, mod.running_mean, mod.running_var, mod.eps, mod.momentum,
                                partials=partials)
        mod.num_batches_tracked += 1
        return st
    return ops.bn_eval_affine(mod.weight, mod.bias, mod.running_mean, mod.running_var, mod.eps)


def _flat2(t):
    return t.view(-1, t.shape[-1])


class _NoGrads:

    def __getitem__(self, _param):
        return None


def _bn_slots(grads, mod: _BatchNorm, st):
    dg, db = grads[mod.weight], grads[mod.bias]
    if dg is None and not st.eval:
        dg, db = torch.empty((2, mod.weight.numel()), dtype=torch.float32, device=mod.weight.device)
    return dg, db


def _w(param):
    words, i = getattr(param, "h2_slot", ([None], 0))
    return ops.Scaled(param, None if words[0] is None else words[0][i:i + 1])


def _res_forward(blk: _ResBlock, x, pool, train, need_grad, slope, x_stats=None, tap=None, frozen=False):
    s = _Ctx()
    s.x = x
    s.bn_pre = _bn(blk.pre_conv[0], x, train, x_stats)
    s.p = ops.bn_act_pool_fwd(x, s.bn_pre, pool=pool, slope=slope, amax_out=True, tap=tap)
    out = ops.gemm_nt(_flat2(s.p), _w(blk.conv1by1.weight).view(blk.cout, blk.cin))
    out = out.view(*s.p.shape[:3], blk.cout)
    wf0, s.wd0 = ops.conv3x3_repack(_w(blk.conv[0].weight), True, need_grad)
    s.c, c_stats = ops.conv3x3_fwd(s.p, wf0, bn_stats=train)
    s.bn_mid = _bn(blk.conv[1], s.c, train, c_stats)
    s.a = ops.bn_act_pool_fwd(s.c, s.bn_mid, pool=1, slope=slope, amax_out=True)
    wf3, s.wd3 = ops.conv3x3_repack(_w(blk.conv[3].weight), True, need_grad)
    _, out_stats = ops.conv3x3_fwd(s.a, wf3, out=out, accumulate=True, bn_stats=train)
    if frozen:
        s.p = s.a = None
    return out, s, out_stats


def _res_backward(blk: _ResBlock, s, d_out, pool, slope, grads, side, tap=None):
    if side is not None:
        side.run(lambda: (ops.conv3x3_wgrad(s.a, d_out, grads[blk.conv[3].weight]),
                          ops.gemm_tn(_flat2(d_out), _flat2(s.p), out=grads[blk.conv1by1.weight].view(blk.cout, blk.cin))),
                 d_out, on=OVERLAP_CONV_WGRAD)
    with ops.timer_tag("dgrad"):
        d_a = ops.conv3x3_fwd(d_out, s.wd3)
    d_c = ops.bn_act_pool_bwd(s.c, d_a, s.bn_mid, *_bn_slots(grads, blk.conv[1], s.bn_mid), pool=1,
                              slope=slope, dx=d_a, amax_out=True)
    if side is not None:
        side.run(lambda: ops.conv3x3_wgrad(s.p, d_c, grads[blk.conv[0].weight]), d_c, on=OVERLAP_CONV_WGRAD)
    with ops.timer_tag("dgrad"):
        d_p = ops.conv3x3_fwd(d_c, s.wd0)
    w1t = ops.transpose2d(_w(blk.conv1by1.weight).view(blk.cout, blk.cin))
    ops.gemm_nt(_flat2(d_out), w1t, out=_flat2(d_p), accumulate=True)
    return ops.bn_act_pool_bwd(s.x, d_p, s.bn_pre, *_bn_slots(grads, blk.pre_conv[0], s.bn_pre),
                               pool=pool, slope=slope, amax_out=True, tap=tap)


class _DropoutCfg:
    def __init__(self, seed=0):
        self.seed = int(seed)
        self.offset = 0
        self.inject = None

    def next_offset(self, n_quads):
        off = self.offset
        self.offset += int(n_quads)
        return off


def _dropout(cfg: _DropoutCfg, x2d, p, out2d=None):
    if p <= 0.0:
        if out2d is not None:
            ops.copy2d(x2d, out2d)
            return out2d, None
        return x2d, None
    mask_in = next(cfg.inject) if cfg.inject is not None else None
# ... 15 lines not shown
    m0 = models[0].model
    H, L, ND = m0.hidden_size, m0.num_layers, m0.num_dirs
    B, T = xs[0].shape[:2]
    saved = []
    cur = list(xs)
    for layer in range(L):
        lay = _Ctx()
        lay.gates, lay.cbuf, lay.y, lay.mask = [], [], [], []
        lay.x = cur = [ops.Scaled.measured(x) if layer == 0 else
                       ops.Scaled.bounded(x, 1.0 / (1.0 - (sm.dropout if train else 0.0))) for x, sm in zip(cur, models)]
        ys = [torch.empty((B, T, ND * H), dtype=torch.float32, device=xs[0].device) for _ in models]
        whh, gts, ysl, cbs, rev = [], [], [], [], []
        for mi, sm in enumerate(models):
            for d in range(ND):
                w_ih, w_hh, b_ih, b_hh = sm.model.cell(layer, d)
                g = ops.gemm_nt(_flat2(cur[mi]), _w(w_ih), bias0=b_ih, bias1=b_hh).view(B, T, 4 * H)
                cb = torch.empty((B, T, H), dtype=torch.float32, device=g.device)
                whh.append(w_hh); gts.append(g); cbs.append(cb); rev.append(d)
                ysl.append(ys[mi][:, :, d * H:(d + 1) * H])
        ops.lstm_fwd(whh, gts, ysl, cbs, rev, B, T, H)
        lay.gates, lay.cbuf, lay.y = gts, cbs, ys
        nxt = []
        for mi, sm in enumerate(models):
            p = sm.dropout if (train and layer < L - 1) else 0.0
            yd, mask = _dropout(drop, _flat2(ys[mi]), p)
            lay.mask.append((p, mask))
            nxt.append(yd.view(B, T, ND * H))
        cur = nxt
        if frozen:
            lay.x = lay.y = None
        saved.append(lay if need_grad else None)
    return cur, saved


OVERLAP_LSTM_WGRAD = os.environ.get("PE_OVERLAP_LSTM_WGRAD", "1") != "0"
_SIDE_STREAMS: dict = {}


def _side_stream(dev):
    key = torch.device(dev)
    if key not in _SIDE_STREAMS:
        stream = None
        if os.environ.get("PE_SIDE_STREAM_PRIORITY", "low") == "low":
            import ctypes
            from . import _lib
            handle = ctypes.c_void_p()
            with torch.cuda.device(key):
                _lib.check(_lib.load().pe_stream_create_low_priority(ctypes.byref(handle)), "pe_stream_create_low_priority")
            stream = torch.cuda.ExternalStream(handle.value, device=key)
        _SIDE_STREAMS[key] = stream if stream is not None else torch.cuda.Stream(device=key)
    return _SIDE_STREAMS[key]


class _SideWork:

    def __init__(self, dev, enabled=True):
        self.dev, self.enabled, self.keep, self.used = dev, enabled, [], False

    def pending_stream(self):
        return _side_stream(self.dev) if self.used else None

    def run(self, fn, *keep, on=True):
        if not (self.enabled and on):
            fn()
            return
        side = _side_stream(self.dev)
        side.wait_stream(torch.cuda.current_stream(self.dev))
        with torch.cuda.stream(side):
            fn()
        self.keep.append(keep)
        self.used = True

    def join(self):
        if self.used:
            torch.cuda.current_stream(self.dev).wait_stream(_side_stream(self.dev))
        self.keep.clear()
        self.used = False


OVERLAP_CONV_WGRAD = os.environ.get("PE_OVERLAP_CONV_WGRAD", "1") != "0"
OVERLAP_TF_WGRAD = os.environ.get("PE_OVERLAP_TF_WGRAD", "1") != "0"
LSTM_WGRAD_JOIN_EARLY = os.environ.get("PE_LSTM_WGRAD_JOIN", "early") == "early"
FOLD_TAPS = os.environ.get("PE_FOLD_TAPS", "1") != "0"


def _lstm_backward(models, saved, dys, grads, side):
    m0 = models[0].model
    H, L, ND = m0.hidden_size, m0.num_layers, m0.num_dirs
    B, T = dys[0].shape[:2]
    dev = dys[0].device
    for layer in reversed(range(L)):
        lay = saved[layer]
        dys = [_dropout_bwd(_flat2(dys[mi]), lay.mask[mi][0], lay.mask[mi][1]).view(B, T, ND * H)
               for mi in range(len(models))]
        whh_t, dsl, dcs, rev = [], [], [], []
        for mi, sm in enumerate(models):
            for d in range(ND):
                _, w_hh, _, _ = sm.model.cell(layer, d)
                whh_t.append(ops.transpose2d(w_hh))
                dsl.append(dys[mi][:, :, d * H:(d + 1) * H])
                dcs.append(torch.empty((B, H), dtype=torch.float32, device=dev))
                rev.append(d)
        nrows = ops.lstm_bwd_dbias_rows(len(whh_t), B, T, H, dsl[0].stride(1), dev)
        brows = [torch.empty((nrows, 4 * H), dtype=torch.float32, device=dev) for _ in whh_t] if nrows else None
        have_db, dgs = ops.lstm_bwd(whh_t, lay.gates, lay.cbuf, dsl, dcs, rev, B, T, H,
                                    dbias_rows=brows, amax_out=True)
        dgs = [ops.Scaled.measured(dg) for dg in dgs]
        dxs = []
        for mi, sm in enumerate(models):
            dx = torch.empty((B, T, sm.model.cell(layer, 0)[0].shape[1]), dtype=torch.float32, device=dev)
            for d in range(ND):
                w_ih = sm.model.cell(layer, d)[0]
                ops.gemm_nt(_flat2(dgs[mi * ND + d]), ops.transpose2d(_w(w_ih)), out=_flat2(dx), accumulate=(d > 0))
            dxs.append(dx)

        def weight_grads(layer=layer, lay=lay, brows=brows, have_db=have_db, dgs=dgs):
            for mi, sm in enumerate(models):
                x2 = _flat2(lay.x[mi])
                for d in range(ND):
                    w_ih, w_hh, b_ih, b_hh = sm.model.cell(layer, d)
                    dg = dgs[mi * ND + d]
                    dg2 = _flat2(dg)
                    ops.gemm_tn(dg2, x2, out=grads[w_ih])
                    ops.lstm_whh_grad(dg, lay.y[mi][:, :, d * H:(d + 1) * H], grads[w_hh], d, B, T, H)
                    ops.colsum(brows[mi * ND + d] if have_db else dg2.t, grads[b_ih], grads[b_hh])

        if side is not None:
            side.run(weight_grads, brows, dgs, on=OVERLAP_LSTM_WGRAD)
        dys = dxs
    return dys


TF_FUSE_DROPOUT = os.environ.get("PE_TF_FUSE_DROPOUT", "1") != "0"


def _mask_or_offset(drop: _DropoutCfg, like):
    mask_in = next(drop.inject) if drop.inject is not None else None
    return mask_in, drop.next_offset(like.numel() // 4)


def _residual_norm(drop: _DropoutCfg, x2d, sub2d, norm, p):
    if p > 0.0 and TF_FUSE_DROPOUT:
        mask_in, off = _mask_or_offset(drop, sub2d)
        return ops.layernorm_dropout_fwd(x2d, sub2d, norm.weight, norm.bias, p, mask_in=mask_in, seed=drop.seed,
                                         offset=off, eps=norm.eps)
    sub2d, mask = _dropout(drop, sub2d, p)
    y, st = ops.layernorm_fwd(x2d, norm.weight, norm.bias, b2d=sub2d, eps=norm.eps)
    return y, st, mask


def _residual_norm_bwd(dy, dy_add, st, norm, g, p, mask):
    if TF_FUSE_DROPOUT:
        if mask is None:
            dsum = ops.layernorm_bwd(dy, st, norm.weight, g[norm.weight], g[norm.bias], dy_add=dy_add)
            return dsum, dsum
        return ops.layernorm_bwd(dy, st, norm.weight, g[norm.weight], g[norm.bias], dy_add=dy_add, drop_mask=mask, p=p)
    if dy_add is not None:
        ops.copy2d(dy_add, dy, accumulate=True)
    dsum = ops.layernorm_bwd(dy, st, norm.weight, g[norm.weight], g[norm.bias])
    return dsum, _dropout_bwd(dsum, p, mask)


def _tf_forward(sm, x, train, need_grad, drop: _DropoutCfg, frozen=False):
    B, T, D = x.shape
    H = sm.nhead
    dh = D // H
# ... 245 lines not shown
            return min(self._param_offsets[id(q)] for q in mod.parameters())

        def last(mod):
            return max(self._param_offsets[id(q)] for q in mod.parameters())
        blocks = [self.conv_block, self.res_block1, self.res_block2, self.res_block3]
        cuts = [first(b) for b in blocks] + [self._seq_offset()]
        tail_ok = all(cuts[3] < first(m) and last(m) < cuts[4] for m in (self.pool_block, self.detector_conv))
        ordered = cuts[0] == 0 and all(a < b for a, b in zip(cuts, cuts[1:])) and \
            all(last(b) < c for b, c in zip(blocks, cuts[1:]))
        return cuts if (ordered and tail_ok) else None

    def _seq_offset(self):
        first = next(self.sequence_classifier.parameters())
        return self._param_offsets[id(first)]

    @property
    def flat_parameters(self) -> torch.Tensor:
        return self._flat

    def flat_gradients(self) -> torch.Tensor:
        if self._grad_flat is None or self._grad_flat.device != self._flat.device:
            self._grad_flat = torch.zeros_like(self._flat, requires_grad=False)
        return self._grad_flat

    def _refresh_weight_amax(self):
        self._wwords[0] = None
        if ops.h2_active() and self._flat is not None and self._flat.is_cuda:
            if getattr(self, "_wseg", None) is None or self._wseg[0].device != self._flat.device:
                offs = torch.tensor([self._param_offsets[id(p)] for p in self._param_list], dtype=torch.int64)
                lens = torch.tensor([p.numel() for p in self._param_list], dtype=torch.int64)
                self._wseg = (offs.to(self._flat.device), lens.to(self._flat.device))
            self._wwords[0] = ops.absmax_segments(self._flat.detach(), self._wseg[0], self._wseg[1])

    scaled = staticmethod(_w)

    def status_slot(self) -> torch.Tensor:
        return self.flat_gradients()[self._status_off:self._status_off + 1]

    def is_frozen(self) -> bool:
        return not any(p.requires_grad for p in self._param_list)

    def _write_status(self, dev, frozen=False):
        word = ops.persistent_lstm_error_word(dev)
        if frozen:
            if self.backward_status is None or self.backward_status.device != torch.device(dev):
                self.backward_status = torch.zeros(1, dtype=torch.float32, device=dev)
            slot = self.backward_status
        else:
            slot = self.status_slot()
        if word is None:
            slot.zero_()
        else:
            slot.copy_(word != 0)

    def _grad_views(self):
        gflat = self.flat_gradients()
        views = {}
        for p in self._param_list:
            off = self._param_offsets[id(p)]
            g = gflat[off:off + p.numel()].view_as(p)
            if p.grad is None or p.grad.data_ptr() != g.data_ptr():
                p.grad = g
            views[p] = g
        return views

    def forward(self, x):
        if not x.is_cuda:
            raise RuntimeError("JDCNet (HIP) needs device tensors; there is no CPU fallback")
        if x.dim() != 4 or x.shape[1] != 1:
            raise ValueError("expected input of shape (B, 1, T, n_mels)")
        frozen = self.is_frozen()
        need_grad = torch.is_grad_enabled() and self.training_graph_wanted and (x.requires_grad or not frozen)
        return _JDCFunction.apply(self, x, None if frozen else self._flat, need_grad)

    def _forward_impl(self, x, need_grad, frozen=False):
        train = self.training
        slope = self.leaky_relu_slope
        self._refresh_weight_amax()
        s = _Ctx()
        x_btf = x[:, 0].float()
        B, T, F = x_btf.shape
        s.x_btf = x_btf
        cbk = self.conv_block
        s.y0, y0_stats = ops.conv3x3_c1_fwd(x_btf, cbk[0].weight, bn_stats=train)
        s.bn0 = _bn(cbk[1], s.y0, train, y0_stats)
        s.a0 = ops.bn_act_pool_fwd(s.y0, s.bn0, pool=1, slope=slope, amax_out=True)
        wf, s.wd_cb = ops.conv3x3_repack(_w(cbk[3].weight), True, need_grad)
        s.cb, st_cb = ops.conv3x3_fwd(s.a0, wf, bn_stats=train)
        s.taps = None
        if FOLD_TAPS:
            s.concat = torch.empty((B, T, 2, 640), dtype=s.cb.dtype, device=x.device)
            s.taps = [ops.Tap(s.concat, tp, coff, want_argmax=need_grad) for tp, coff in ((40, 0), (20, 64), (10, 192))]
        t_cb, t_rb1, t_rb2 = s.taps or (None, None, None)
        s.rb1, s.r1, st1 = _res_forward(self.res_block1, s.cb, 2, train, need_grad, slope, st_cb, t_cb, frozen)
        s.rb2, s.r2, st2 = _res_forward(self.res_block2, s.rb1, 2, train, need_grad, slope, st1, t_rb1, frozen)
        s.rb3, s.r3, st3 = _res_forward(self.res_block3, s.rb2, 2, train, need_grad, slope, st2, t_rb2, frozen)

        Fp = s.rb3.shape[2] // 4
        if Fp != 2:
            raise ValueError("JDCNet geometry expects 80 mel bins (F/40 == 2)")
        s.bnp = _bn(self.pool_block[0], s.rb3, train, st3)
        pooled = ops.bn_act_pool_fwd(s.rb3, s.bnp, pool=4, slope=slope)
        if s.taps is None:
            s.concat = torch.empty((B, T, 2, 640), dtype=s.rb3.dtype, device=x.device)
        p_blk = self.block_dropout if train else 0.0
        cslice = s.concat.view(-1, 640)[:, 384:640]
        _, s.mask_pool = _dropout(self.dropout_cfg, _flat2(pooled), p_blk, out2d=cslice)
        seq_c = ops.nhwc_to_seq(s.concat, 256, coff=384)

        if s.taps is None:
            _, s.arg_cb = ops.maxpool_fwd(s.cb, 40, out=s.concat, coff=0, want_argmax=True)
            _, s.arg_rb1 = ops.maxpool_fwd(s.rb1, 20, out=s.concat, coff=64, want_argmax=True)
            _, s.arg_rb2 = ops.maxpool_fwd(s.rb2, 10, out=s.concat, coff=192, want_argmax=True)
        s.dconv = ops.gemm_nt(s.concat.view(-1, 640), _w(self.detector_conv[0].weight).view(256, 640))
        s.dconv = s.dconv.view(B, T, 2, 256)
        s.bnd = _bn(self.detector_conv[1], s.dconv, train)
        dact = ops.bn_act_pool_fwd(s.dconv, s.bnd, pool=1, slope=slope)
        ddrop, s.mask_det = _dropout(self.dropout_cfg, _flat2(dact), p_blk)
        seq_d = ops.nhwc_to_seq(ddrop.view(B, T, 2, 256), 256)

        models = [self.sequence_classifier, self.sequence_detector]
        if models[0].model_type == "bilstm":
            (yc, yd), s.lstm = _lstm_forward(models, [seq_c, seq_d], train, need_grad, self.dropout_cfg, frozen)
        else:
            yc, s.tf_c = _tf_forward(models[0], seq_c, train, need_grad, self.dropout_cfg, frozen)
            yd, s.tf_d = _tf_forward(models[1], seq_d, train, need_grad, self.dropout_cfg, frozen)
        s.yc, s.yd = yc, yd
        D = yc.shape[-1]
        if self.num_class == 1:
            out_cls = ops.head_fwd(yc.view(-1, D), self.classifier.weight, self.classifier.bias).view(B, T, 1)
        else:
            out_cls = ops.gemm_nt(yc.view(-1, D), self.classifier.weight, bias0=self.classifier.bias)
            out_cls = out_cls.view(B, T, self.num_class)
        out_det = ops.head_fwd(yd.view(-1, D), self.detector.weight, self.detector.bias).view(B, T)
        s.shape = (B, T, F)
        s.frozen, s.act_dtype = frozen, s.concat.dtype
        if frozen:
            s.x_btf = s.a0 = s.concat = None
            for t in s.taps or ():
                t.out = None
        return out_cls, out_det, (s if need_grad else None)

    def _backward_impl(self, s, d_cls, d_det, want_dx=False):
        frozen = s.frozen
        g = _NoGrads() if frozen else self._grad_views()
        dp = None if frozen else self._dp
        slope = self.leaky_relu_slope
        B, T, F = s.shape
        D = s.yc.shape[-1]
        dev = s.yc.device
        if d_cls is None:
            d_cls = torch.zeros((B, T, self.num_class), dtype=torch.float32, device=dev)
        if d_det is None:
            d_det = torch.zeros((B, T), dtype=torch.float32, device=dev)
        d_cls = d_cls.contiguous().float()
        d_det = d_det.contiguous().float()
        cls, det = self.classifier, self.detector
        if self.num_class == 1:
            dyc = ops.head_bwd(s.yc.view(-1, D), cls.weight, d_cls.view(-1), g[cls.weight], g[cls.bias])
        else:
            d2 = d_cls.view(-1, self.num_class)
            if not frozen:
                ops.gemm_tn(d2, s.yc.view(-1, D), out=g[cls.weight])
                ops.colsum(d2, g[cls.bias])
            dyc = ops.gemm_nt(d2, ops.transpose2d(cls.weight))
        dyd = ops.head_bwd(s.yd.view(-1, D), det.weight, d_det.view(-1), g[det.weight], g[det.bias])

        models = [self.sequence_classifier, self.sequence_detector]
        side = None if frozen else _SideWork(dev)
        if models[0].model_type == "bilstm":
            dseq_c, dseq_d = _lstm_backward(models, s.lstm, [dyc.view(B, T, D), dyd.view(B, T, D)], g, side)
            if LSTM_WGRAD_JOIN_EARLY and side is not None:
                side.join()
        else:
            dseq_d = _tf_backward(models[1], s.tf_d, dyd.view(B, T, D), g, side)
            dseq_c = _tf_backward(models[0], s.tf_c, dyc.view(B, T, D), g, side)

        self._write_status(dev, frozen)
        if dp is not None:
            dp.reduce_range(self._seq_offset(), self._grad_flat.numel(), after=side.pending_stream())

        p_blk = self.block_dropout
        d_ddrop = torch.empty((B, T, 2, 256), dtype=s.act_dtype, device=dev)
        ops.seq_to_nhwc(dseq_d, d_ddrop, 256)
        d_dact = _dropout_bwd(_flat2(d_ddrop), p_blk, s.mask_det).view(B, T, 2, 256)
        bn1 = self.detector_conv[1]
        d_dconv = ops.bn_act_pool_bwd(s.dconv, d_dact, s.bnd, *_bn_slots(g, bn1, s.bnd), pool=1, slope=slope)
        wdet = self.detector_conv[0].weight
        if side is not None:
            side.run(lambda: ops.gemm_tn(_flat2(d_dconv), s.concat.view(-1, 640), out=g[wdet].view(256, 640)), d_dconv,
                     on=OVERLAP_CONV_WGRAD)
        d_concat = ops.gemm_nt(_flat2(d_dconv), ops.transpose2d(_w(wdet).view(256, 640)))
        d_concat = d_concat.view(B, T, 2, 640)
        ops.seq_to_nhwc(dseq_c, d_concat, 256, coff=384, accumulate=True)
        d_pool = torch.empty((B, T, 2, 256), dtype=s.act_dtype, device=dev)
        _dropout_bwd(d_concat.view(-1, 640)[:, 384:640], p_blk if s.mask_pool is not None else 0.0, s.mask_pool,
                     out2d=_flat2(d_pool))
        bnp = self.pool_block[0]
        d_rb3 = ops.bn_act_pool_bwd(s.rb3, d_pool, s.bnp, *_bn_slots(g, bnp, s.bnp), pool=4, slope=slope, amax_out=True)

        cuts = self._dp_cuts if dp is not None else None

        def block_done(k):
            if cuts is not None:
                dp.reduce_range(cuts[k], cuts[k + 1], after=side.pending_stream())

        t_cb, t_rb1, t_rb2 = s.taps or (None, None, None)
        for t in s.taps or ():
            t.grad = d_concat
        d_rb2 = _res_backward(self.res_block3, s.r3, d_rb3, 2, slope, g, side, t_rb2)
        block_done(3)
        if s.taps is None:
            d_rb2 = ops.maxpool_bwd_add(s.rb2, d_concat, d_rb2, 10, coff=192, argmax=s.arg_rb2)
        d_rb1 = _res_backward(self.res_block2, s.r2, d_rb2, 2, slope, g, side, t_rb1)
        block_done(2)
        if s.taps is None:
            d_rb1 = ops.maxpool_bwd_add(s.rb1, d_concat, d_rb1, 20, coff=64, argmax=s.arg_rb1)
        d_cb = _res_backward(self.res_block1, s.r1, d_rb1, 2, slope, g, side, t_cb)
        block_done(1)
        if s.taps is None:
            d_cb = ops.maxpool_bwd_add(s.cb, d_concat, d_cb, 40, coff=0, argmax=s.arg_cb)

        cbk = self.conv_block
        if side is not None:
            side.run(lambda: ops.conv3x3_wgrad(s.a0, d_cb, g[cbk[3].weight]), d_cb, on=OVERLAP_CONV_WGRAD)
        with ops.timer_tag("dgrad"):
            d_a0 = ops.conv3x3_fwd(d_cb, s.wd_cb)
        d_y0 = ops.bn_act_pool_bwd(s.y0, d_a0, s.bn0, *_bn_slots(g, cbk[1], s.bn0), pool=1, slope=slope, dx=d_a0)
        if not frozen:
            ops.conv3x3_c1_wgrad(s.x_btf, d_y0, g[cbk[0].weight])
        dx = ops.conv3x3_c1_dgrad(d_y0, cbk[0].weight) if want_dx else None
        if side is not None:
            side.join()
        if dp is not None:
            dp.reduce_range(0, cuts[1] if cuts is not None else self._seq_offset())
        return dx
```

### pitchextractor_amd/ops.py

```python
from __future__ import annotations

import ctypes as C

import os

import torch

from . import _lib

_WS: dict = {}


def _chk(cond, msg):
    if not cond:
        raise ValueError(msg)


def _f32c(t: torch.Tensor, name: str) -> torch.Tensor:
    _chk(t.is_cuda, f"{name}: expected a HIP device tensor (no CPU fallback)")
    _chk(t.dtype == torch.float32, f"{name}: expected float32")
    return t


def _dense(t: torch.Tensor, name: str) -> torch.Tensor:
# ... 350 lines not shown
        elif CONV_WFRAG and p != _lib.PE_PROD_NATIVE and t.shape[1] % 16 == 0:
            out.append(PackedWeight(Scaled(t, amax), wfrag_pack(Scaled(t, amax), p), p))
        else:
            out.append(PackedWeight(Scaled(t, amax)))
    return out[0], out[1]


def conv3x3_fwd(x, w_packed, out=None, accumulate=False, bn_stats=None):
    x, amax = _tw(x)
    x = _actd(x, "x")
    pw = w_packed if isinstance(w_packed, PackedWeight) else PackedWeight(w_packed)
    w32 = _dense(pw.fp32, "w_packed")
    _chk(x.dim() == 4 and w32.dim() == 2, "conv3x3_fwd: ranks")
    B, T, F, Cc = x.shape
    N = w32.shape[0]
    _chk(w32.shape[1] == 9 * Cc, "conv3x3_fwd: weight K")
    if out is None:
        _chk(not accumulate, "accumulate needs out")
        out = torch.empty((B, T, F, N), dtype=x.dtype, device=x.device)
    _chk(_actd(out, "out").shape == (B, T, F, N), "conv3x3_fwd: out shape")
    p, a16 = products_for(), _act16(x, out)
    _chk(not a16 or p == _lib.PE_PROD_BF16, "bfloat16 activations need the bf16 mixed-precision mode")
    amax_w = None
    if p == _lib.PE_PROD_H2:
        amax_w = pw.amax if pw.amax is not None else absmax(w32)
        amax = absmax(x) if amax is None else amax
    h2 = (_lib.ptr(amax), _lib.ptr(amax_w))
    work = 2.0 * B * T * F * N * 9 * Cc
    if pw.frag is not None and pw.products == p and CONV_WFRAG and _lib.load().pe_conv3x3_wf_supported(F, Cc, N):
        parts = None
        if bn_stats:
            parts = torch.empty((_lib.load().pe_conv3x3_wf_stat_parts(B, T, F), 2, N), dtype=torch.float64,
                                device=x.device)
        _call("pe_conv3x3_fwd_wf", x.data_ptr(), pw.frag.data_ptr(), out.data_ptr(), B, T, F, Cc, N,
              int(bool(accumulate)), _lib.ptr(parts), *h2, _s(), products=p, act16=a16, work=work)
        return (out, parts) if bn_stats is not None else out
    _call("pe_conv3x3_fwd", x.data_ptr(), w32.data_ptr(), out.data_ptr(), B, T, F, Cc, N, int(bool(accumulate)), *h2,
          _s(), products=p, act16=a16, work=work)
    return (out, None) if bn_stats is not None else out


def conv3x3_wgrad(x, dy, dw):
    (x, amax_x), (dy, amax_dy) = _tw(x), _tw(dy)
    x = _actd(x, "x")
    dy = _actd(dy, "dy")
    dw = _dense(dw, "dw")
    B, T, F, Ci = x.shape
    Co = dy.shape[3]
    _chk(dy.shape[:3] == (B, T, F), "conv3x3_wgrad: dy shape")
    _chk(dw.shape == (Co, Ci, 3, 3), "conv3x3_wgrad: dw shape")
    p, a16 = products_for(), _act16(x, dy)
    _chk(not a16 or p == _lib.PE_PROD_BF16, "bfloat16 activations need the bf16 mixed-precision mode")
    ws = workspace(_lib.load().pe_conv3x3_wgrad_workspace_bytes(B, T, F, Ci, Co), x.device)
    if p == _lib.PE_PROD_H2:
        amax_x = absmax(x) if amax_x is None else amax_x
        amax_dy = absmax(dy) if amax_dy is None else amax_dy
    _call("pe_conv3x3_wgrad", x.data_ptr(), dy.data_ptr(), dw.data_ptr(), B, T, F, Ci, Co, ws.data_ptr(), ws.numel(),
          _lib.ptr(amax_x), _lib.ptr(amax_dy), _s(), products=p, act16=a16, work=2.0 * B * T * F * Co * 9 * Ci)
    return dw


def _btf_view(x):
    _f32c(x, "x")
    _chk(x.dim() == 3, "expected (B,T,F)")
    return x.shape, x.stride()


def conv3x3_c1_fwd(x_btf, w, out=None, bn_stats=None):
    (B, T, F), (sb, st, sf) = _btf_view(x_btf)
    w = _dense(w, "w")
    _chk(w.shape == (64, 1, 3, 3), "first conv is 1 -> 64")
    if out is None:
        out = torch.empty((B, T, F, 64), dtype=act_dtype(), device=x_btf.device)
    _chk(_actd(out, "out").shape == (B, T, F, 64), "conv3x3_c1_fwd: out shape")
    parts = None
    if bn_stats:
        parts = torch.empty((_lib.load().pe_conv3x3_c1_stat_parts(B, T, F), 2, 64), dtype=torch.float64,
                            device=x_btf.device)
    _call("pe_conv3x3_c1_fwd", x_btf.data_ptr(), sb, st, sf, w.data_ptr(), out.data_ptr(), B, T, F, _lib.ptr(parts), _s(),
          act16=_act16(out))
    return out if bn_stats is None else (out, parts)


def conv3x3_c1_wgrad(x_btf, dy, dw):
    (B, T, F), (sb, st, sf) = _btf_view(x_btf)
    dy = _actd(dy, "dy")
    dw = _dense(dw, "dw")
    _chk(dy.shape == (B, T, F, 64) and dw.shape == (64, 1, 3, 3), "conv3x3_c1_wgrad: shapes")
    lib = _lib.load()
    ws = workspace(lib.pe_conv3x3_wgrad_workspace_bytes(B, T, F, 1, 64), dy.device)
    _call("pe_conv3x3_c1_wgrad", x_btf.data_ptr(), sb, st, sf, dy.data_ptr(), dw.data_ptr(), B, T, F, ws.data_ptr(),
          ws.numel(), _s(), act16=_act16(dy))
    return dw


def conv3x3_c1_dgrad(dy, w, out=None):
    _chk(dy.is_cuda and dy.is_contiguous() and dy.dim() == 4 and dy.shape[3] == 64 and dy.dtype in _DGRAD_ACT,
         "conv3x3_c1_dgrad: dy must be a dense [B,T,F,64] float32 / bfloat16 / float16 device tensor")
    w = _dense(w, "w")
    _chk(w.shape == (64, 1, 3, 3) and w.device == dy.device, "first conv is 1 -> 64")
    B, T, F = dy.shape[:3]
    if out is None:
        out = torch.empty((B, T, F), dtype=torch.float32, device=dy.device)
    _chk(_dense(out, "out").shape == (B, T, F) and out.device == dy.device, "conv3x3_c1_dgrad: out shape")
    a16 = _DGRAD_ACT[dy.dtype]
    _call("pe_conv3x3_c1_dgrad", a16, dy.data_ptr(), w.data_ptr(), out.data_ptr(), B, T, F, _s(),
          work=2.0 * B * T * F * 576, key="pe_conv3x3_c1_dgrad" + ("_a16" if a16 else ""))
    return out


_DGRAD_ACT = {torch.float32: 0, torch.bfloat16: 1, torch.float16: 2}


class BnState:

    def __init__(self, C_, device, eval=False):
        buf = torch.empty((4, C_), dtype=torch.float32, device=device)
        self.mean, self.invstd, self.scale, self.shift = buf[0], buf[1], buf[2], buf[3]
        self.eval = bool(eval)


def bn_train_stats(x, gamma, beta, running_mean, running_var, eps=1e-5, momentum=0.1, partials=None):
    x = _actd(x, "x")
    Cc = x.shape[-1]
    for t, n in ((gamma, "gamma"), (beta, "beta"), (running_mean, "running_mean"), (running_var, "running_var")):
        if t is not None:
            _chk(_dense(t, n).numel() == Cc, f"{n}: size")
    st = BnState(Cc, x.device)
    lib = _lib.load()
    if partials is not None:
        _chk(partials.is_cuda and partials.dtype == torch.float64 and partials.is_contiguous() and partials.dim() == 3
             and partials.shape[1:] == (2, Cc), "bn_train_stats: partials [parts, 2, C] float64")
        ws = workspace(lib.pe_bn_workspace_bytes(Cc), x.device)
        _call("pe_bn_finalize_stats", partials.data_ptr(), partials.shape[0], x.numel() // Cc, Cc, gamma.data_ptr(),
              beta.data_ptr(), eps, momentum, _lib.ptr(running_mean), _lib.ptr(running_var), st.mean.data_ptr(),
              st.invstd.data_ptr(), st.scale.data_ptr(), st.shift.data_ptr(), ws.data_ptr(), ws.numel(), _s())
        return st
    ws = workspace(lib.pe_bn_workspace_bytes(Cc), x.device)
    _call("pe_bn_train_stats", x.data_ptr(), x.numel() // Cc, Cc, gamma.data_ptr(), beta.data_ptr(), eps, momentum,
          _lib.ptr(running_mean), _lib.ptr(running_var), st.mean.data_ptr(), st.invstd.data_ptr(),
          st.scale.data_ptr(), st.shift.data_ptr(), ws.data_ptr(), ws.numel(), _s(), act16=_act16(x))
    return st


def bn_eval_affine(gamma, beta, running_mean, running_var, eps=1e-5):
    Cc = gamma.numel()
    st = BnState(Cc, gamma.device, eval=True)
    for t in (gamma, beta, running_mean, running_var):
        _chk(_dense(t, "bn tensor").numel() == Cc, "bn tensor size")
    _call("pe_bn_eval_affine", gamma.data_ptr(), beta.data_ptr(), running_mean.data_ptr(), running_var.data_ptr(),
          eps, Cc, st.scale.data_ptr(), st.shift.data_ptr(), st.mean.data_ptr(), st.invstd.data_ptr(), _s())
    return st


def _slice_target(out, B, T, Fo, Cc, coff):
    _actd(out, "out")
    _chk(out.dim() == 4 and out.shape[:3] == (B, T, Fo), "output pixel grid mismatch")
    ld = out.shape[3]
    _chk(0 <= coff and coff + Cc <= ld, "channel slice out of range")
    return ld


class Tap:

    def __init__(self, out, pool, coff, want_argmax=False):
        self.out, self.pool, self.coff, self.want_argmax = out, int(pool), int(coff), bool(want_argmax)
        self.argmax = None
        self.grad = None


def _tap_folded(x, pool, tap: Tap, with_arg) -> bool:
    B, T, F, Cc = x.shape
    return bool(_lib.load().pe_bn_act_pool_tap_supported(B * T, F, Cc, pool, tap.pool, int(with_arg)))


def bn_act_pool_fwd(x, st: BnState, pool=1, slope=0.01, out=None, coff=0, amax_out=None, tap: Tap | None = None):
    x = _actd(x, "x")
    paired, amax_out = amax_out is True, (amax_word() if amax_out is True else amax_out)
    B, T, F, Cc = x.shape
    Fo = F // pool
    if out is None:
        out = torch.empty((B, T, Fo, Cc), dtype=x.dtype, device=x.device)
    ld = _slice_target(out, B, T, Fo, Cc, coff)
    if tap is not None and _tap_folded(x, pool, tap, tap.want_argmax):
        Ft = F // tap.pool
        tld = _slice_target(tap.out, B, T, Ft, Cc, tap.coff)
        tap.argmax = torch.empty((B, T, Ft, Cc), dtype=torch.uint8, device=x.device) if tap.want_argmax else None
        _call("pe_bn_act_pool_tap_fwd", x.data_ptr(), st.scale.data_ptr(), st.shift.data_ptr(), slope, out.data_ptr(),
              B * T, F, Cc, pool, ld, coff, _lib.ptr(amax_out), tap.out.data_ptr(), tld, tap.coff, tap.pool,
              _lib.ptr(tap.argmax), _s(), act16=_act16(x, out, tap.out))
        return Scaled(out, amax_out) if paired else out
    _call("pe_bn_act_pool_fwd", x.data_ptr(), st.scale.data_ptr(), st.shift.data_ptr(), slope, out.data_ptr(),
          B * T, F, Cc, pool, ld, coff, _lib.ptr(amax_out), _s(), act16=_act16(x, out))
    if tap is not None:
        if tap.want_argmax:
            _, tap.argmax = maxpool_fwd(x, tap.pool, out=tap.out, coff=tap.coff, want_argmax=True)
        else:
            maxpool_fwd(x, tap.pool, out=tap.out, coff=tap.coff)
    return Scaled(out, amax_out) if paired else out


def bn_act_pool_bwd(x, dy, st: BnState, dgamma, dbeta, pool=1, slope=0.01, coff=0, dx=None, amax_out=None,
                    tap: Tap | None = None):
    x = _actd(x, "x")
    _chk(pool in (1, 2, 4), "bn_act_pool_bwd: pool is 1, 2 or 4")
    paired, amax_out = amax_out is True, (amax_word() if amax_out is True else amax_out)
    B, T, F, Cc = x.shape
    ld = _slice_target(dy, B, T, F // pool, Cc, coff)
    if dx is None:
        dx = torch.empty_like(x)
    _chk(_actd(dx, "dx").shape == x.shape, "dx shape")
    ev = int(st.eval)
    if dgamma is None and dbeta is None:
        _chk(st.eval, "bn_act_pool_bwd: only an eval-mode BatchNorm has an input gradient without dgamma / dbeta")
        ws_ptr, ws_len = None, 0
    else:
        _chk(_dense(dgamma, "dgamma").numel() == Cc and _dense(dbeta, "dbeta").numel() == Cc, "dgamma/dbeta size")
        ws = workspace(_lib.load().pe_bn_workspace_bytes(Cc) + 8 * Cc, x.device)
        ws_ptr, ws_len = ws.data_ptr(), ws.numel()
    if tap is not None and tap.argmax is not None and _tap_folded(x, pool, tap, True):
        Ft = F // tap.pool
        _chk(tap.argmax.is_cuda and tap.argmax.dtype == torch.uint8 and tap.argmax.is_contiguous()
# ... 670 lines not shown
```

Measured before the change: 655,600.

## Recompute first 1->64 conv inside BN/act and backward kernels instead of storing it

The first convolution (1 input channel to 64) is no longer written out as a 64-channel pre-BN tensor. The forward pass runs a stats-only conv pass, then a fused kernel that recomputes the conv and applies BN and leaky ReLU. In backward, a sums kernel and the wgrad kernel each recompute the conv output from the single-channel input, so BN backward is fused into wgrad and can write dx in place. This trades several full-resolution 64-channel reads and writes for extra cheap conv arithmetic, but adds one additional pass over the input in forward and in backward.

```diff
diff --git a/include/pitchextractor_hip.h b/include/pitchextractor_hip.h
--- a/include/pitchextractor_hip.h
+++ b/include/pitchextractor_hip.h
@@ -89,8 +89,12 @@
 int pe_conv3x3_c1_stat_parts(int B, int T, int F);
 int pe_conv3x3_c1_fwd(int act16, const float* x, long sb, long st, long sf, const float* w_oihw, void* y, int B, int T,
                       int F, double* bn_partials, void* stream);
-int pe_conv3x3_c1_wgrad(int act16, const float* x, long sb, long st, long sf, const void* dy, float* dw_oihw, int B,
-                        int T, int F, float* workspace, size_t workspace_bytes, void* stream);
+int pe_conv3x3_c1_stats(int act16, const float* x, long sb, long st, long sf, const float* w_oihw, int B, int T, int F,
+                        double* bn_partials, void* stream);
+int pe_conv3x3_c1_wgrad(int act16, const float* x, long sb, long st, long sf, void* dy, float* dw_oihw, int B, int T,
+                        int F, float* workspace, size_t workspace_bytes, void* stream, const float* bn_w,
+                        const float* bn_scale, const float* bn_shift, const float* bn_mean, const float* bn_invstd,
+                        const float* bn_k, float slope, int store_dy);
 int pe_conv3x3_c1_dgrad(int act16, const void* dy, const float* w_oihw, float* dx, int B, int T, int F, void* stream);
 
 int pe_attn_supported(int T, int dh);
@@ -118,6 +122,12 @@
                        const float* mean, const float* invstd, float slope, void* dx, float* dgamma, float* dbeta,
                        long rows, int Fin, int C, int pool, long lddy, int coff, int eval_mode, void* workspace,
                        size_t workspace_bytes, unsigned* amax_out, void* stream);
+int pe_c1_bn_act_fwd(int act16, const float* x, long sb, long st, long sf, const float* w_oihw, const float* scale,
+                     const float* shift, float slope, void* y, int B, int T, int F, unsigned* amax_out, void* stream);
+int pe_c1_bn_bwd_sums(int act16, const float* x, long sb, long st, long sf, const float* w_oihw, const void* dy,
+                      const float* scale, const float* shift, const float* mean, const float* invstd, float slope,
+                      float* dgamma, float* dbeta, float* bn_k, int B, int T, int F, void* workspace,
+                      size_t workspace_bytes, void* stream);
 int pe_maxpool_fwd(int act16, const void* x, void* y, long rows, int Fin, int C, int pool, long ldy, int coff,
                    unsigned char* argmax_out, void* stream);
 int pe_maxpool_bwd_add(int act16, const void* x, const unsigned char* argmax, const void* dy, void* dx, long rows,
diff --git a/pitchextractor_amd/_lib.py b/pitchextractor_amd/_lib.py
--- a/pitchextractor_amd/_lib.py
+++ b/pitchextractor_amd/_lib.py
@@ -60,7 +60,10 @@
     "pe_conv3x3_wgrad": (_i, [_i, _i, _p, _p, _p, _i, _i, _i, _i, _i, _p, _z, _p, _p, _p]),
     "pe_conv3x3_c1_stat_parts": (_i, [_i, _i, _i]),
     "pe_conv3x3_c1_fwd": (_i, [_i, _p, _l, _l, _l, _p, _p, _i, _i, _i, _p, _p]),
-    "pe_conv3x3_c1_wgrad": (_i, [_i, _p, _l, _l, _l, _p, _p, _i, _i, _i, _p, _z, _p]),
+    "pe_conv3x3_c1_stats": (_i, [_i, _p, _l, _l, _l, _p, _i, _i, _i, _p, _p]),
+    "pe_conv3x3_c1_wgrad": (_i, [_i, _p, _l, _l, _l, _p, _p, _i, _i, _i, _p, _z, _p, _p, _p, _p, _p, _p, _p, _f, _i]),
+    "pe_c1_bn_act_fwd": (_i, [_i, _p, _l, _l, _l, _p, _p, _p, _f, _p, _i, _i, _i, _p, _p]),
+    "pe_c1_bn_bwd_sums": (_i, [_i, _p, _l, _l, _l, _p, _p, _p, _p, _p, _p, _f, _p, _p, _p, _i, _i, _i, _p, _z, _p]),
     "pe_conv3x3_c1_dgrad": (_i, [_i, _p, _p, _p, _i, _i, _i, _p]),
     "pe_bn_workspace_bytes": (_z, [_i]),
     "pe_bn_train_stats": (_i, [_i, _p, _l, _i, _p, _p, _f, _f, _p, _p, _p, _p, _p, _p, _p, _z, _p]),
diff --git a/pitchextractor_amd/csrc/conv.hip b/pitchextractor_amd/csrc/conv.hip
--- a/pitchextractor_amd/csrc/conv.hip
+++ b/pitchextractor_amd/csrc/conv.hip
@@ -1,4 +1,5 @@
 #include <type_traits>
+#include "first_layer.h"
 #include "splitk.h"
 
 namespace {
@@ -45,11 +46,6 @@
   }
 };
 typedef ConvEpiT<float> ConvEpi;
-
-template <class TO> __device__ __forceinline__ float stored_value(float v) {
-  if constexpr (std::is_same<TO, float>::value) return v;
-  else return __uint_as_float(pack_bf16_rne(v, 0.f) << 16);
-}
 
 template <class TL, int MODE, class TA = float, class TH = __bf16>
 __global__ __launch_bounds__(256) void conv3x3_kernel(ConvLoader<TL::A_LOADS, TA> al, RowLoader bl, ConvEpiT<TA> ep,
@@ -685,48 +681,36 @@
                      tn, n_tiles, n_chunks);
 }
 
-template <bool STATS, class TA = float>
+template <bool STATS, class TA = float, bool STORE = true>
 __global__ __launch_bounds__(256) void conv3x3_c1_fwd_kernel(const float* __restrict__ x, long sb, long st_, long sf,
                                                              const float* __restrict__ w, TA* __restrict__ y,
                                                              double* __restrict__ bn_partials, int B, int T, int F) {
+  static_assert(STATS || STORE, "a kernel with nothing to leave behind");
   __shared__ double sred[STATS ? 2 * 16 * 64 : 1];
   double s1[4] = {0.0, 0.0, 0.0, 0.0}, s2[4] = {0.0, 0.0, 0.0, 0.0};
   const int q = threadIdx.x & 15;
   float wr[4][9];
-#pragma unroll
-  for (int c = 0; c < 4; ++c)
-#pragma unroll
-    for (int k = 0; k < 9; ++k) wr[c][k] = w[(q * 4 + c) * 9 + k];
+  c1_load_weights(w, q, wr);
   const int F4 = F >> 2, R = B * T * F4;
   for (int run = blockIdx.x * 16 + (threadIdx.x >> 4); run < R; run += gridDim.x * 16) {
     const int bt = run / F4, f0 = (run - bt * F4) * 4;
     const long b = bt / T;
     const int t = bt - (int)b * T;
     float in[3][6];
-#pragma unroll
-    for (int dt = 0; dt < 3; ++dt)
-#pragma unroll
-      for (int df = 0; df < 6; ++df) {
-        const int tt = t + dt - 1, ff = f0 + df - 1;
-        in[dt][df] = (tt >= 0 && tt < T && ff >= 0 && ff < F) ? x[b * sb + tt * st_ + ff * sf] : 0.f;
-      }
+    c1_load_run(x + b * sb, st_, sf, t, f0, T, F, in);
 #pragma unroll
     for (int px = 0; px < 4; ++px) {
-      float4 o;
-      float* op = reinterpret_cast<float*>(&o);
-#pragma unroll
-      for (int c = 0; c < 4; ++c) {
-        float s = 0.f;
-#pragma unroll
-        for (int k = 0; k < 9; ++k) s = fmaf(in[k / 3][px + k % 3], wr[c][k], s);
-        op[c] = s;
-        if constexpr (STATS) {
-          const double dv = (double)stored_value<TA>(s);
+      const float4 o = c1_quad(wr, [&](int k) { return in[k / 3][px + k % 3]; });
+      if constexpr (STATS) {
+        const float* op = reinterpret_cast<const float*>(&o);
+#pragma unroll
+        for (int c = 0; c < 4; ++c) {
+          const double dv = (double)stored_value<TA>(op[c]);
           s1[c] += dv;
           s2[c] += dv * dv;
         }
       }
-      st4(y + ((long)bt * F + f0 + px) * 64 + q * 4, o);
+      if constexpr (STORE) st4(y + ((long)bt * F + f0 + px) * 64 + q * 4, o);
     }
   }
   if constexpr (STATS) {
@@ -747,10 +731,22 @@
   }
 }
 
-template <class TA = float>
+struct C1BnGrad {
+  const float* w;
+  const float* scale;
+  const float* shift;
+  const float* mean;
+  const float* invstd;
+  const float* k1;
+  const float* k2;
+  float slope;
+};
+
+template <class TA = float, int MODE = 0>
 __global__ __launch_bounds__(256) void conv3x3_c1_wgrad_kernel(const float* __restrict__ x, long sb, long st_,
                                                                long sf, const TA* __restrict__ dy,
-                                                               float* __restrict__ partial, int B, int T, int F) {
+                                                               float* __restrict__ partial, int B, int T, int F,
+                                                               const C1BnGrad bn, TA* dy_io) {
   __shared__ float red[16][64][9];
   const int q = threadIdx.x & 15, grp = threadIdx.x >> 4;
   float acc[4][9];
@@ -758,21 +754,31 @@
   for (int c = 0; c < 4; ++c)
 #pragma unroll
     for (int k = 0; k < 9; ++k) acc[c][k] = 0.f;
+  [[maybe_unused]] float wr[4][9];
+  [[maybe_unused]] float4 mu, is, sc, sh, k1, k2;
+  if constexpr (MODE != 0) {
+    c1_load_weights(bn.w, q, wr);
+    mu = *reinterpret_cast<const float4*>(bn.mean + q * 4), is = *reinterpret_cast<const float4*>(bn.invstd + q * 4);
+    sc = *reinterpret_cast<const float4*>(bn.scale + q * 4), sh = *reinterpret_cast<const float4*>(bn.shift + q * 4);
+    k1 = *reinterpret_cast<const float4*>(bn.k1 + q * 4), k2 = *reinterpret_cast<const float4*>(bn.k2 + q * 4);
+  }
   const int F4 = F >> 2, R = B * T * F4;
   for (int run = blockIdx.x * 16 + grp; run < R; run += gridDim.x * 16) {
     const int bt = run / F4, f0 = (run - bt * F4) * 4, b = bt / T, t = bt - b * T;
-    const float* xb = x + b * sb;
     float in[3][6];
-#pragma unroll
-    for (int dt = 0; dt < 3; ++dt)
-#pragma unroll
-      for (int df = 0; df < 6; ++df) {
-        const int tt = t + dt - 1, ff = f0 + df - 1;
-        in[dt][df] = (tt >= 0 && tt < T && ff >= 0 && ff < F) ? xb[tt * st_ + ff * sf] : 0.f;
-      }
+    c1_load_run(x + b * sb, st_, sf, t, f0, T, F, in);
 #pragma unroll
     for (int px = 0; px < 4; ++px) {
-      const float4 g = ld4(dy + ((long)bt * F + f0 + px) * 64 + q * 4);
+      const long at = ((long)bt * F + f0 + px) * 64 + q * 4;
+      float4 g;
+      if constexpr (MODE == 0) {
+        g = ld4(dy + at);
+      } else {
+        const float4 v = c1_stored<TA>(c1_quad(wr, [&](int k) { return in[k / 3][px + k % 3]; }));
+        const float4 o = bn_dx4(bn_lrelu_dz4(v, ld4(dy_io + at), sc, sh, bn.slope), v, mu, is, sc, k1, k2);
+        if constexpr (MODE == 2) st4(dy_io + at, o);
+        g = make_float4(round_act(dy_io, o.x), round_act(dy_io, o.y), round_act(dy_io, o.z), round_act(dy_io, o.w));
+      }
 #pragma unroll
       for (int k = 0; k < 9; ++k) {
         const float xv = in[k / 3][px + k % 3];
@@ -1035,11 +1041,6 @@
   });
 }
 
-static int c1_grid(int B, int T, int F) {
-  const long R = (long)B * T * (F / 4);
-  return (int)((R + 15) / 16 < 8192 ? (R + 15) / 16 : 8192);
-}
-
 extern "C" int pe_conv3x3_c1_stat_parts(int B, int T, int F) { return (B > 0 && T > 0 && F > 0) ? c1_grid(B, T, F) : 0; }
 
 template <class TA>
@@ -1066,27 +1067,55 @@
   });
 }
 
+extern "C" int pe_conv3x3_c1_stats(int act16, const float* x, long sb, long st, long sf, const float* w_oihw, int B, int T,
+                                   int F, double* bn_partials, void* stream) {
+  if (!x || !w_oihw || !bn_partials) return PE_E_ARG;
+  if (const int e = c1_geometry_status(B, T, F)) return e;
+  return with_act(act16, [&](auto a) {
+    using TA = typename decltype(a)::TA;
+    hipLaunchKernelGGL((conv3x3_c1_fwd_kernel<true, TA, false>), dim3(c1_grid(B, T, F)), dim3(256), 0, pe_stream(stream),
+                       x, sb, st, sf, w_oihw, static_cast<TA*>(nullptr), bn_partials, B, T, F);
+    PE_LAUNCH_CHECK();
+    return (int)PE_OK;
+  });
+}
+
 template <class TA>
 static int conv3x3_c1_wgrad_impl(const float* x, long sb, long st, long sf, const TA* dy, float* dw_oihw, int B, int T,
-                                 int F, float* workspace, size_t workspace_bytes, void* stream) {
+                                 int F, float* workspace, size_t workspace_bytes, const C1BnGrad* bn, int store_dy,
+                                 void* stream) {
   if (!x || !dy || !dw_oihw || B <= 0 || T <= 0 || F <= 0) return PE_E_ARG;
   if ((F & 3) || (long)B * T * F >= (1L << 31) - 65536) return PE_E_UNSUPPORTED;
   if (!workspace || workspace_bytes < (size_t)kC1WgradBlocks * 576 * sizeof(float)) return PE_E_WORKSPACE;
-  hipLaunchKernelGGL(conv3x3_c1_wgrad_kernel<TA>, dim3(kC1WgradBlocks), dim3(256), 0, pe_stream(stream), x, sb, st, sf,
-                     dy, workspace, B, T, F);
+  const dim3 grid(kC1WgradBlocks), block(256);
+  hipStream_t s = pe_stream(stream);
+  TA* io = const_cast<TA*>(dy);
+  if (bn == nullptr)
+    hipLaunchKernelGGL((conv3x3_c1_wgrad_kernel<TA, 0>), grid, block, 0, s, x, sb, st, sf, dy, workspace, B, T, F,
+                       C1BnGrad{}, static_cast<TA*>(nullptr));
+  else if (store_dy)
+    hipLaunchKernelGGL((conv3x3_c1_wgrad_kernel<TA, 2>), grid, block, 0, s, x, sb, st, sf,
+                       static_cast<const TA*>(nullptr), workspace, B, T, F, *bn, io);
+  else
+    hipLaunchKernelGGL((conv3x3_c1_wgrad_kernel<TA, 1>), grid, block, 0, s, x, sb, st, sf,
+                       static_cast<const TA*>(nullptr), workspace, B, T, F, *bn, io);
   PE_LAUNCH_CHECK();
-  hipLaunchKernelGGL(c1_wgrad_reduce_kernel, dim3(144), dim3(256), 0, pe_stream(stream), workspace, dw_oihw,
-                     kC1WgradBlocks);
+  hipLaunchKernelGGL(c1_wgrad_reduce_kernel, dim3(144), dim3(256), 0, s, workspace, dw_oihw, kC1WgradBlocks);
   PE_LAUNCH_CHECK();
   return PE_OK;
 }
 
-extern "C" int pe_conv3x3_c1_wgrad(int act16, const float* x, long sb, long st, long sf, const void* dy, float* dw_oihw,
-                                   int B, int T, int F, float* workspace, size_t workspace_bytes, void* stream) {
+extern "C" int pe_conv3x3_c1_wgrad(int act16, const float* x, long sb, long st, long sf, void* dy, float* dw_oihw, int B,
+                                   int T, int F, float* workspace, size_t workspace_bytes, void* stream,
+                                   const float* bn_w, const float* bn_scale, const float* bn_shift,
+                                   const float* bn_mean, const float* bn_invstd, const float* bn_k, float slope,
+                                   int store_dy) {
+  if (bn_w && (!bn_scale || !bn_shift || !bn_mean || !bn_invstd || !bn_k)) return PE_E_ARG;
+  const C1BnGrad bn{bn_w, bn_scale, bn_shift, bn_mean, bn_invstd, bn_k, bn_k ? bn_k + 64 : nullptr, slope};
   return with_act(act16, [&](auto a) {
     using TA = typename decltype(a)::TA;
     return conv3x3_c1_wgrad_impl(x, sb, st, sf, static_cast<const TA*>(dy), dw_oihw, B, T, F, workspace, workspace_bytes,
-                                 stream);
+                                 bn_w ? &bn : nullptr, store_dy, stream);
   });
 }
 
diff --git a/pitchextractor_amd/csrc/elementwise.hip b/pitchextractor_amd/csrc/elementwise.hip
--- a/pitchextractor_amd/csrc/elementwise.hip
+++ b/pitchextractor_amd/csrc/elementwise.hip
@@ -1,4 +1,5 @@
 #include <type_traits>
+#include "first_layer.h"
 #include "forms.h"
 
 namespace {
@@ -35,21 +36,8 @@
   }
 }
 
-__device__ __forceinline__ float lrelu(float v, float slope) { return v > 0.f ? v : v * slope; }
-
-__device__ __forceinline__ float4 bn_lrelu4(const float4& v, const float4& sc, const float4& sh, float slope) {
-  return make_float4(lrelu(fmaf(v.x, sc.x, sh.x), slope), lrelu(fmaf(v.y, sc.y, sh.y), slope),
-                     lrelu(fmaf(v.z, sc.z, sh.z), slope), lrelu(fmaf(v.w, sc.w, sh.w), slope));
-}
-
 __device__ __forceinline__ float4 fmax4(const float4& a, const float4& b) {
   return make_float4(fmaxf(a.x, b.x), fmaxf(a.y, b.y), fmaxf(a.z, b.z), fmaxf(a.w, b.w));
-}
-
-__device__ __forceinline__ float4 bn_dx4(const float4& dz, const float4& v, const float4& mu, const float4& is,
-                                         const float4& sc, const float4& k1, const float4& k2) {
-  return make_float4(sc.x * (dz.x - k1.x - (v.x - mu.x) * is.x * k2.x), sc.y * (dz.y - k1.y - (v.y - mu.y) * is.y * k2.y),
-                     sc.z * (dz.z - k1.z - (v.z - mu.z) * is.z * k2.z), sc.w * (dz.w - k1.w - (v.w - mu.w) * is.w * k2.w));
 }
 
 __device__ __forceinline__ void first_max(float& m, int& at, float x, int pos, bool force = false) {
@@ -191,6 +179,36 @@
     }
     st4(y + op * ldy + coff + q * 4, m);
     am = amax4(am, m);
+  }
+  amax_commit(am, amax);
+}
+
+template <class TA>
+__global__ __launch_bounds__(256) void c1_bn_act_fwd_kernel(const float* __restrict__ x, long sb, long st_, long sf,
+                                                            const float* __restrict__ w,
+                                                            const float* __restrict__ scale,
+                                                            const float* __restrict__ shift, float slope,
+                                                            TA* __restrict__ y, int B, int T, int F,
+                                                            unsigned* __restrict__ amax) {
+  const int q = threadIdx.x & 15;
+  float wr[4][9];
+  c1_load_weights(w, q, wr);
+  const float4 sc = *reinterpret_cast<const float4*>(scale + q * 4), sh = *reinterpret_cast<const float4*>(shift + q * 4);
+  float am = 0.f;
+  const int F4 = F >> 2, R = B * T * F4;
+  for (int run = blockIdx.x * 16 + (threadIdx.x >> 4); run < R; run += gridDim.x * 16) {
+    const int bt = run / F4, f0 = (run - bt * F4) * 4;
+    const long b = bt / T;
+    const int t = bt - (int)b * T;
+    float in[3][6];
+    c1_load_run(x + b * sb, st_, sf, t, f0, T, F, in);
+#pragma unroll
+    for (int px = 0; px < 4; ++px) {
+      const float4 v = c1_stored<TA>(c1_quad(wr, [&](int k) { return in[k / 3][px + k % 3]; }));
+      const float4 m = bn_lrelu4(v, sc, sh, slope);
+      st4(y + ((long)bt * F + f0 + px) * 64 + q * 4, m);
+      am = amax4(am, m);
+    }
   }
   amax_commit(am, amax);
 }
@@ -358,6 +376,37 @@
 }
 
 template <class TA>
+__global__ __launch_bounds__(256) void c1_bn_bwd_partial_kernel(const float* __restrict__ x, long sb, long st_,
+                                                                long sf, const float* __restrict__ w,
+                                                                const BnBwdArgsT<TA> a, int T,
+                                                                double* __restrict__ partial) {
+  const int q = threadIdx.x & 15, c0 = q * 4;
+  const float4 mu = *reinterpret_cast<const float4*>(a.mean + c0), is = *reinterpret_cast<const float4*>(a.invstd + c0);
+  const float4 sc = *reinterpret_cast<const float4*>(a.scale + c0), sh = *reinterpret_cast<const float4*>(a.shift + c0);
+  float wr[4][9];
+  c1_load_weights(w, q, wr);
+  const int F = a.Fin, dt = q / 3 - 1, df = q % 3 - 1;
+  const int first = threadIdx.x & 48;
+  column_reduce2(
+      [&](long p, int c, float4& s, float4& t) {
+        const int pw = __builtin_amdgcn_readfirstlane((int)p), row = pw / F, b = row / T, tt = row - b * T;
+        const int f = pw - row * F + (first >> 4);
+        const float mine = q < 9 ? c1_input(x + b * sb, st_, sf, tt + dt, f + df, T, F) : 0.f;
+        float in[9];
+#pragma unroll
+        for (int k = 0; k < 9; ++k) in[k] = __shfl(mine, first + k, 64);
+        const float4 v = c1_stored<TA>(c1_quad(wr, [&](int k) { return in[k]; }));
+        const float4 dz = bn_lrelu_dz4(v, ld4(a.dy + p * a.lddy + a.coff + c), sc, sh, a.slope);
+        s = make_float4(0.f, 0.f, 0.f, 0.f);
+        t = make_float4(0.f, 0.f, 0.f, 0.f);
+        s.x += dz.x; s.y += dz.y; s.z += dz.z; s.w += dz.w;
+        t.x += dz.x * ((v.x - mu.x) * is.x); t.y += dz.y * ((v.y - mu.y) * is.y);
+        t.z += dz.z * ((v.z - mu.z) * is.z); t.w += dz.w * ((v.w - mu.w) * is.w);
+      },
+      a.n_in_pix, 64, partial);
+}
+
+template <class TA>
 struct BnTapGrad {
   const TA* dy;
   const unsigned char* arg;
@@ -366,10 +415,6 @@
   unsigned nbw;
 };
 
-__device__ __forceinline__ float round_act(const float*, float v) { return v; }
-__device__ __forceinline__ float round_act(const act16_t*, float v) {
-  return __uint_as_float(pack_bf16_rne(v, 0.f) << 16);
-}
 __device__ __forceinline__ float add_unfused(float a, float b) {
 #pragma clang fp contract(off)
   return a + b;
@@ -792,6 +837,44 @@
   });
 }
 
+extern "C" int pe_c1_bn_act_fwd(int act16, const float* x, long sb, long st, long sf, const float* w_oihw,
+                                const float* scale, const float* shift, float slope, void* y, int B, int T, int F,
+                                unsigned* amax_out, void* stream) {
+  if (!x || !w_oihw || !scale || !shift || !y) return PE_E_ARG;
+  if (const int e = c1_geometry_status(B, T, F)) return e;
+  return with_act(act16, [&](auto a) {
+    using TA = typename decltype(a)::TA;
+    hipLaunchKernelGGL(c1_bn_act_fwd_kernel<TA>, dim3(c1_grid(B, T, F)), dim3(256), 0, pe_stream(stream), x, sb, st, sf,
+                       w_oihw, scale, shift, slope, static_cast<TA*>(y), B, T, F, amax_out);
+    PE_LAUNCH_CHECK();
+    return (int)PE_OK;
+  });
+}
+
+extern "C" int pe_c1_bn_bwd_sums(int act16, const float* x, long sb, long st, long sf, const float* w_oihw,
+                                 const void* dy, const float* scale, const float* shift, const float* mean,
+                                 const float* invstd, float slope, float* dgamma, float* dbeta, float* bn_k, int B,
+                                 int T, int F, void* workspace, size_t workspace_bytes, void* stream) {
+  if (!x || !w_oihw || !dy || !scale || !shift || !mean || !invstd || !dgamma || !dbeta || !bn_k) return PE_E_ARG;
+  if (const int e = c1_geometry_status(B, T, F)) return e;
+  if (!workspace || workspace_bytes < pe_bn_workspace_bytes(64)) return PE_E_WORKSPACE;
+  return with_act(act16, [&](auto act) {
+    using TA = typename decltype(act)::TA;
+    const long n_pix = (long)B * T * F;
+    const BnBwdArgsT<TA> a{nullptr, static_cast<const TA*>(dy), scale, shift, mean, invstd, slope, n_pix, F, 64, 64, 0};
+    hipStream_t s = pe_stream(stream);
+    double* partial = reinterpret_cast<double*>(workspace);
+    const int grid = reduce_grid(n_pix, 64, std::is_same<TA, float>::value ? 1024 : kMaxPartials);
+    hipLaunchKernelGGL(c1_bn_bwd_partial_kernel<TA>, dim3(grid), dim3(256), reduce_lds(64), s, x, sb, st, sf, w_oihw, a,
+                       T, partial);
+    PE_LAUNCH_CHECK();
+    hipLaunchKernelGGL(bn_bwd_finalize_kernel, dim3(16), dim3(256), 0, s, partial, grid, n_pix, 64, dgamma, dbeta, bn_k,
+                       bn_k + 64);
+    PE_LAUNCH_CHECK();
+    return (int)PE_OK;
+  });
+}
+
 static bool tap_geometry_ok(long rows, int Fin, int C, int pool, int tap_pool, bool with_arg) {
   if (!bn_channels_ok(C) || rows <= 0 || Fin <= 0) return false;
   if (pool != 1 && pool != 2 && pool != 4) return false;
diff --git a/pitchextractor_amd/csrc/first_layer.h b/pitchextractor_amd/csrc/first_layer.h
--- /dev/null
+++ b/pitchextractor_amd/csrc/first_layer.h
@@ -0,0 +1,85 @@
+#pragma once
+#include <type_traits>
+#include "act16.h"
+
+namespace pe {
+
+template <class TO> __device__ __forceinline__ float stored_value(float v) {
+  if constexpr (std::is_same<TO, float>::value) return v;
+  else return __uint_as_float(pack_bf16_rne(v, 0.f) << 16);
+}
+
+__device__ __forceinline__ float round_act(const float*, float v) { return v; }
+__device__ __forceinline__ float round_act(const act16_t*, float v) {
+  return __uint_as_float(pack_bf16_rne(v, 0.f) << 16);
+}
+
+__device__ __forceinline__ float lrelu(float v, float slope) { return v > 0.f ? v : v * slope; }
+
+__device__ __forceinline__ float4 bn_lrelu4(const float4& v, const float4& sc, const float4& sh, float slope) {
+  return make_float4(lrelu(fmaf(v.x, sc.x, sh.x), slope), lrelu(fmaf(v.y, sc.y, sh.y), slope),
+                     lrelu(fmaf(v.z, sc.z, sh.z), slope), lrelu(fmaf(v.w, sc.w, sh.w), slope));
+}
+
+__device__ __forceinline__ float4 bn_dx4(const float4& dz, const float4& v, const float4& mu, const float4& is,
+                                         const float4& sc, const float4& k1, const float4& k2) {
+  return make_float4(sc.x * (dz.x - k1.x - (v.x - mu.x) * is.x * k2.x), sc.y * (dz.y - k1.y - (v.y - mu.y) * is.y * k2.y),
+                     sc.z * (dz.z - k1.z - (v.z - mu.z) * is.z * k2.z), sc.w * (dz.w - k1.w - (v.w - mu.w) * is.w * k2.w));
+}
+
+__device__ __forceinline__ float4 bn_lrelu_dz4(const float4& v, const float4& dy, const float4& sc, const float4& sh,
+                                               float slope) {
+  const float4 a = bn_lrelu4(v, sc, sh, slope);
+  return make_float4(a.x > 0.f ? dy.x : dy.x * slope, a.y > 0.f ? dy.y : dy.y * slope, a.z > 0.f ? dy.z : dy.z * slope,
+                     a.w > 0.f ? dy.w : dy.w * slope);
+}
+
+__device__ __forceinline__ void c1_load_weights(const float* __restrict__ w, int q, float (&wr)[4][9]) {
+#pragma unroll
+  for (int c = 0; c < 4; ++c)
+#pragma unroll
+    for (int k = 0; k < 9; ++k) wr[c][k] = w[(q * 4 + c) * 9 + k];
+}
+
+__device__ __forceinline__ float c1_input(const float* __restrict__ xb, long st_, long sf, int t, int f, int T, int F) {
+  return (t >= 0 && t < T && f >= 0 && f < F) ? xb[t * st_ + f * sf] : 0.f;
+}
+
+__device__ __forceinline__ void c1_load_run(const float* __restrict__ xb, long st_, long sf, int t, int f0, int T, int F,
+                                            float (&in)[3][6]) {
+#pragma unroll
+  for (int dt = 0; dt < 3; ++dt)
+#pragma unroll
+    for (int df = 0; df < 6; ++df) in[dt][df] = c1_input(xb, st_, sf, t + dt - 1, f0 + df - 1, T, F);
+}
+
+template <class Tap>
+__device__ __forceinline__ float4 c1_quad(const float (&wr)[4][9], Tap&& tap) {
+  float o[4];
+#pragma unroll
+  for (int c = 0; c < 4; ++c) {
+    float s = 0.f;
+#pragma unroll
+    for (int k = 0; k < 9; ++k) s = fmaf(tap(k), wr[c][k], s);
+    o[c] = s;
+  }
+  return make_float4(o[0], o[1], o[2], o[3]);
+}
+
+template <class TA>
+__device__ __forceinline__ float4 c1_stored(const float4& o) {
+  return make_float4(stored_value<TA>(o.x), stored_value<TA>(o.y), stored_value<TA>(o.z), stored_value<TA>(o.w));
+}
+
+static inline int c1_grid(int B, int T, int F) {
+  const long R = (long)B * T * (F / 4);
+  return (int)((R + 15) / 16 < 8192 ? (R + 15) / 16 : 8192);
+}
+
+static inline int c1_geometry_status(int B, int T, int F) {
+  if (B <= 0 || T <= 0 || F <= 0) return PE_E_ARG;
+  if ((F & 3) || (long)B * T * F >= (1L << 31) - 64L * 8192) return PE_E_UNSUPPORTED;
+  return PE_OK;
+}
+
+}
diff --git a/pitchextractor_amd/csrc/lib.hip b/pitchextractor_amd/csrc/lib.hip
--- a/pitchextractor_amd/csrc/lib.hip
+++ b/pitchextractor_amd/csrc/lib.hip
@@ -1,6 +1,6 @@
 #include "common.h"
 
-extern "C" int pe_abi_version(void) { return 7; }
+extern "C" int pe_abi_version(void) { return 8; }
 
 extern "C" int pe_device_count(void) {
   int n = 0;
diff --git a/pitchextractor_amd/model.py b/pitchextractor_amd/model.py
--- a/pitchextractor_amd/model.py
+++ b/pitchextractor_amd/model.py
@@ -159,10 +159,10 @@
     """Tensors one forward pass leaves behind for its backward."""
 
 
-def _bn(mod: _BatchNorm, x, train: bool, partials=None):
+def _bn(mod: _BatchNorm, x, train: bool, partials=None, n_pix=None):
     if train:
         st = ops.bn_train_stats(x, mod.weight, mod.bias, mod.running_mean, mod.running_var, mod.eps, mod.momentum,
-                                partials=partials)
+                                partials=partials, n_pix=n_pix)
         mod.num_batches_tracked += 1
         return st
     return ops.bn_eval_affine(mod.weight, mod.bias, mod.running_mean, mod.running_var, mod.eps)
@@ -344,6 +344,7 @@
 OVERLAP_TF_WGRAD = os.environ.get("PE_OVERLAP_TF_WGRAD", "1") != "0"
 LSTM_WGRAD_JOIN_EARLY = os.environ.get("PE_LSTM_WGRAD_JOIN", "early") == "early"
 FOLD_TAPS = os.environ.get("PE_FOLD_TAPS", "1") != "0"
+C1_RECOMPUTE = os.environ.get("PE_C1_RECOMPUTE", "1") != "0"
 
 
 def _lstm_backward(models, saved, dys, grads, side):
@@ -755,9 +756,18 @@
         B, T, F = x_btf.shape
         s.x_btf = x_btf
         cbk = self.conv_block
-        s.y0, y0_stats = ops.conv3x3_c1_fwd(x_btf, cbk[0].weight, bn_stats=train)
-        s.bn0 = _bn(cbk[1], s.y0, train, y0_stats)
-        s.a0 = ops.bn_act_pool_fwd(s.y0, s.bn0, pool=1, slope=slope, amax_out=True)
+        s.y0 = None
+        recompute = C1_RECOMPUTE and ops.act_dtype() == torch.float32
+        if recompute and ((train and not frozen) or (not train and not need_grad)):
+            if train:
+                s.bn0 = _bn(cbk[1], None, True, ops.conv3x3_c1_stats(x_btf, cbk[0].weight), n_pix=B * T * F)
+            else:
+                s.bn0 = _bn(cbk[1], None, False)
+            s.a0 = ops.c1_bn_act_fwd(x_btf, cbk[0].weight, s.bn0, slope=slope, amax_out=True)
+        else:
+            s.y0, y0_stats = ops.conv3x3_c1_fwd(x_btf, cbk[0].weight, bn_stats=train)
+            s.bn0 = _bn(cbk[1], s.y0, train, y0_stats)
+            s.a0 = ops.bn_act_pool_fwd(s.y0, s.bn0, pool=1, slope=slope, amax_out=True)
         wf, s.wd_cb = ops.conv3x3_repack(_w(cbk[3].weight), True, need_grad)
         s.cb, st_cb = ops.conv3x3_fwd(s.a0, wf, bn_stats=train)
         s.taps = None
@@ -899,9 +909,14 @@
             side.run(lambda: ops.conv3x3_wgrad(s.a0, d_cb, g[cbk[3].weight]), d_cb, on=OVERLAP_CONV_WGRAD)
         with ops.timer_tag("dgrad"):
             d_a0 = ops.conv3x3_fwd(d_cb, s.wd_cb)
-        d_y0 = ops.bn_act_pool_bwd(s.y0, d_a0, s.bn0, *_bn_slots(g, cbk[1], s.bn0), pool=1, slope=slope, dx=d_a0)
-        if not frozen:
-            ops.conv3x3_c1_wgrad(s.x_btf, d_y0, g[cbk[0].weight])
+        if s.y0 is None:
+            rc = ops.c1_bn_bwd_sums(s.x_btf, cbk[0].weight, d_a0, s.bn0, *_bn_slots(g, cbk[1], s.bn0), slope=slope)
+            ops.conv3x3_c1_wgrad(s.x_btf, d_a0, g[cbk[0].weight], bn=rc, store_dy=want_dx)
+            d_y0 = d_a0
+        else:
+            d_y0 = ops.bn_act_pool_bwd(s.y0, d_a0, s.bn0, *_bn_slots(g, cbk[1], s.bn0), pool=1, slope=slope, dx=d_a0)
+            if not frozen:
+                ops.conv3x3_c1_wgrad(s.x_btf, d_y0, g[cbk[0].weight])
         dx = ops.conv3x3_c1_dgrad(d_y0, cbk[0].weight) if want_dx else None
         if side is not None:
             side.join()
diff --git a/pitchextractor_amd/ops.py b/pitchextractor_amd/ops.py
--- a/pitchextractor_amd/ops.py
+++ b/pitchextractor_amd/ops.py
@@ -456,15 +456,68 @@
     return out if bn_stats is None else (out, parts)
 
 
-def conv3x3_c1_wgrad(x_btf, dy, dw):
+def _c1_operands(x_btf, w, name):
+    (B, T, F), strides = _btf_view(x_btf)
+    w = _dense(w, "w")
+    _chk(w.shape == (64, 1, 3, 3) and w.device == x_btf.device, f"{name}: first conv is 1 -> 64")
+    return (B, T, F), strides
+
+
+def conv3x3_c1_stats(x_btf, w):
+    (B, T, F), (sb, st, sf) = _c1_operands(x_btf, w, "conv3x3_c1_stats")
+    parts = torch.empty((_lib.load().pe_conv3x3_c1_stat_parts(B, T, F), 2, 64), dtype=torch.float64, device=x_btf.device)
+    _call("pe_conv3x3_c1_stats", x_btf.data_ptr(), sb, st, sf, w.data_ptr(), B, T, F, parts.data_ptr(), _s(),
+          act16=act_dtype() == torch.bfloat16)
+    return parts
+
+
+def c1_bn_act_fwd(x_btf, w, st: "BnState", slope=0.01, out=None, amax_out=None):
+    (B, T, F), (sb, s_t, sf) = _c1_operands(x_btf, w, "c1_bn_act_fwd")
+    paired, amax_out = amax_out is True, (amax_word() if amax_out is True else amax_out)
+    if out is None:
+        out = torch.empty((B, T, F, 64), dtype=act_dtype(), device=x_btf.device)
+    _chk(_actd(out, "out").shape == (B, T, F, 64) and out.device == x_btf.device, "c1_bn_act_fwd: out shape")
+    _call("pe_c1_bn_act_fwd", x_btf.data_ptr(), sb, s_t, sf, w.data_ptr(), st.scale.data_ptr(), st.shift.data_ptr(),
+          slope, out.data_ptr(), B, T, F, _lib.ptr(amax_out), _s(), act16=_act16(out))
+    return Scaled(out, amax_out) if paired else out
+
+
+class C1Recompute:
+
+    def __init__(self, w, st: "BnState", k, slope=0.01):
+        self.w, self.st, self.k, self.slope = w, st, k, float(slope)
+
+
+def c1_bn_bwd_sums(x_btf, w, dy, st: "BnState", dgamma, dbeta, slope=0.01) -> C1Recompute:
+    (B, T, F), (sb, s_t, sf) = _c1_operands(x_btf, w, "c1_bn_bwd_sums")
+    _chk(not st.eval, "c1_bn_bwd_sums: batch statistics only")
+    _chk(_actd(dy, "dy").shape == (B, T, F, 64) and dy.device == x_btf.device, "c1_bn_bwd_sums: dy shape")
+    _chk(_dense(dgamma, "dgamma").numel() == 64 and _dense(dbeta, "dbeta").numel() == 64, "dgamma/dbeta size")
+    k = torch.empty((2, 64), dtype=torch.float32, device=dy.device)
+    ws = workspace(_lib.load().pe_bn_workspace_bytes(64), dy.device)
+    _call("pe_c1_bn_bwd_sums", x_btf.data_ptr(), sb, s_t, sf, w.data_ptr(), dy.data_ptr(), st.scale.data_ptr(),
+          st.shift.data_ptr(), st.mean.data_ptr(), st.invstd.data_ptr(), slope, dgamma.data_ptr(), dbeta.data_ptr(),
+          k.data_ptr(), B, T, F, ws.data_ptr(), ws.numel(), _s(), act16=_act16(dy))
+    return C1Recompute(w, st, k, slope)
+
+
+def conv3x3_c1_wgrad(x_btf, dy, dw, bn: C1Recompute | None = None, store_dy=False):
     (B, T, F), (sb, st, sf) = _btf_view(x_btf)
     dy = _actd(dy, "dy")
     dw = _dense(dw, "dw")
     _chk(dy.shape == (B, T, F, 64) and dw.shape == (64, 1, 3, 3), "conv3x3_c1_wgrad: shapes")
     lib = _lib.load()
     ws = workspace(lib.pe_conv3x3_wgrad_workspace_bytes(B, T, F, 1, 64), dy.device)
+    if bn is None:
+        _chk(not store_dy, "conv3x3_c1_wgrad: store_dy needs bn")
+        extra = (None, None, None, None, None, None, 0.0, 0)
+    else:
+        _chk(_dense(bn.w, "bn.w").shape == (64, 1, 3, 3) and _dense(bn.k, "bn.k").shape == (2, 64)
+             and bn.st.mean.numel() == 64 and bn.w.device == bn.k.device == dy.device, "conv3x3_c1_wgrad: bn operands")
+        extra = (bn.w.data_ptr(), bn.st.scale.data_ptr(), bn.st.shift.data_ptr(), bn.st.mean.data_ptr(),
+                 bn.st.invstd.data_ptr(), bn.k.data_ptr(), bn.slope, int(bool(store_dy)))
     _call("pe_conv3x3_c1_wgrad", x_btf.data_ptr(), sb, st, sf, dy.data_ptr(), dw.data_ptr(), B, T, F, ws.data_ptr(),
-          ws.numel(), _s(), act16=_act16(dy))
+          ws.numel(), _s(), *extra, act16=_act16(dy))
     return dw
 
 
@@ -494,24 +547,28 @@
         self.eval = bool(eval)
 
 
-def bn_train_stats(x, gamma, beta, running_mean, running_var, eps=1e-5, momentum=0.1, partials=None):
-    x = _actd(x, "x")
-    Cc = x.shape[-1]
+def bn_train_stats(x, gamma, beta, running_mean, running_var, eps=1e-5, momentum=0.1, partials=None, n_pix=None):
+    if x is None:
+        _chk(partials is not None and n_pix is not None, "bn_train_stats: no tensor needs partials and n_pix")
+        Cc, dev = gamma.numel(), gamma.device
+    else:
+        x = _actd(x, "x")
+        Cc, dev, n_pix = x.shape[-1], x.device, x.numel() // x.shape[-1]
     for t, n in ((gamma, "gamma"), (beta, "beta"), (running_mean, "running_mean"), (running_var, "running_var")):
         if t is not None:
             _chk(_dense(t, n).numel() == Cc, f"{n}: size")
-    st = BnState(Cc, x.device)
+    st = BnState(Cc, dev)
     lib = _lib.load()
     if partials is not None:
         _chk(partials.is_cuda and partials.dtype == torch.float64 and partials.is_contiguous() and partials.dim() == 3
              and partials.shape[1:] == (2, Cc), "bn_train_stats: partials [parts, 2, C] float64")
-        ws = workspace(lib.pe_bn_workspace_bytes(Cc), x.device)
-        _call("pe_bn_finalize_stats", partials.data_ptr(), partials.shape[0], x.numel() // Cc, Cc, gamma.data_ptr(),
+        ws = workspace(lib.pe_bn_workspace_bytes(Cc), dev)
+        _call("pe_bn_finalize_stats", partials.data_ptr(), partials.shape[0], n_pix, Cc, gamma.data_ptr(),
               beta.data_ptr(), eps, momentum, _lib.ptr(running_mean), _lib.ptr(running_var), st.mean.data_ptr(),
               st.invstd.data_ptr(), st.scale.data_ptr(), st.shift.data_ptr(), ws.data_ptr(), ws.numel(), _s())
         return st
-    ws = workspace(lib.pe_bn_workspace_bytes(Cc), x.device)
-    _call("pe_bn_train_stats", x.data_ptr(), x.numel() // Cc, Cc, gamma.data_ptr(), beta.data_ptr(), eps, momentum,
+    ws = workspace(lib.pe_bn_workspace_bytes(Cc), dev)
+    _call("pe_bn_train_stats", x.data_ptr(), n_pix, Cc, gamma.data_ptr(), beta.data_ptr(), eps, momentum,
           _lib.ptr(running_mean), _lib.ptr(running_var), st.mean.data_ptr(), st.invstd.data_ptr(),
           st.scale.data_ptr(), st.shift.data_ptr(), ws.data_ptr(), ws.numel(), _s(), act16=_act16(x))
     return st
```

After: 661,400, median of 6. Within noise of the previous version (+0.9%).
